# zju3dv/RelightableAvatar

Hardware: AMD Instinct MI355X
Metric: rays_per_sec (higher is better)
Workload: dtype f16

## Files before the change

### include/relightableavatar.h

```cpp
#ifndef RELIGHTABLEAVATAR_H
#define RELIGHTABLEAVATAR_H

#include <stddef.h>
#include <stdint.h>

#ifdef __cplusplus
extern "C" {
#endif

#define RA_ABI_VERSION 9
#define RA_N_LIGHTS_MAX 512

typedef struct ra_ctx ra_ctx;

const char* ra_last_error(void);
int ra_abi_version(void);

int ra_ctx_create(ra_ctx** out, int device);
int ra_ctx_destroy(ra_ctx* ctx);

typedef struct ra_config {
    int   xyz_res, sdf_res, view_res;
    int   n_bones;
    int   relight;
// ... 97 lines not shown
    int   no_visibility, local_visibility;
    int   premultiply;
    int   n_boxes;
    const float* boxes;
    const int*   box_start;
} ra_sphere_params;

int ra_render_sphere_chunk(ra_ctx* ctx, const float* ray_o, const float* ray_d, const float* near_,
                           const float* far_, int P, const float* bbox_host6,
                           const float* probe_dev, int probe_h, int probe_w,
                           const ra_sphere_params* p, const ra_render_out* out, void* stream);

int ra_gather_rays(int device, const long long* idx_dev, int n, const float* ray_o, const float* ray_d, const float* near_, const float* far_,
                   float* out_o, float* out_d, float* out_near, float* out_far, void* stream);

int ra_scatter_rows(int device, const float* src_dev, const long long* src_idx_dev, const long long* dst_idx_dev, long long n, int C,
                    float* dst_dev, void* stream);

int ra_begin_render(ra_ctx* ctx);

int ra_set_key_probes(ra_ctx* ctx, const float* probes_dev, int n, int probe_h, int probe_w, int accumulate, void* stream);

int ra_set_light_xyz(ra_ctx* ctx, const float* xyz_dev, void* stream);

int ra_light_visibility(ra_ctx* ctx, const float* surf, const float* norm, const float* acc, int n, const int* rows_dev, int n_rows,
                        const float* bbox_host6, const float* probe_dev, int probe_h, int probe_w, const ra_sphere_params* params,
                        float* lvis, float* ldot, void* stream);

int ra_render_volume_chunk(ra_ctx* ctx, const float* ray_o, const float* ray_d, const float* near_,
                           const float* far_, int P, int n_samples, float dist_th,
                           const ra_render_out* out, void* stream);

int ra_reshade(ra_ctx* ctx, const float* ray_o, const float* surf, const float* norm,
               const float* albedo, const float* roughness, const float* lvis, const float* ldot,
               int P, const float* probes_dev, int n_probes, int probe_h, int probe_w,
               float* rgb, float* shade, float* spec, void* stream);

int ra_reshade_backward(ra_ctx* ctx, const float* ray_o, const float* surf, const float* norm,
                        const float* albedo, const float* roughness, const float* lvis, const float* ldot, int P,
                        const float* probes_dev, int n_probes, int probe_h, int probe_w,
                        const float* d_rgb, float* d_albedo, float* d_roughness, float* d_probes, void* stream);

size_t ra_heads_param_count(const ra_ctx* ctx);
int ra_heads_get_params(ra_ctx* ctx, float* theta_dev, void* stream);
int ra_heads_forward(ra_ctx* ctx, const float* theta_dev, const float* feat_dev, int n, float* albedo_dev, float* rough_dev, void* stream);
int ra_heads_backward(ra_ctx* ctx, const float* theta_dev, const float* feat_dev, int n,
                      const float* d_albedo_dev, const float* d_rough_dev, float* d_theta_dev, void* stream);
int ra_bigpose_features(ra_ctx* ctx, const float* bpts_dev, int n, float* feat_dev, void* stream);

int ra_canonical_features(ra_ctx* ctx, const float* cpts_dev, int n, float* feat_dev, void* stream);
int ra_gaussian_entropy(ra_ctx* ctx, const float* x_dev, int n, const float* d_value_dev, float* value_dev, float* d_x_dev, void* stream);

int ra_reshade_ground(ra_ctx* ctx, const float* ray_d, const float* albedo_map, const float* lvis, const float* ldot, int P,
                      const float* probes_dev, int n_probes, int probe_h, int probe_w, const float* images_dev, int image_h, int image_w,
                      int attach_envmap, float* rgb, float* albedo, float* shade, float* spec, void* stream);

typedef struct ra_counters {
    uint64_t n_coarse;
    uint64_t n_fine_sdf;
    uint64_t n_fine_full;
    uint64_t n_shadow_rays;
    uint64_t n_hit_pixels;
    uint64_t n_shaded;
    uint64_t n_fine_sdf_wide;
    uint64_t n_fine_sdf_comp;
} ra_counters;
int ra_get_counters(ra_ctx* ctx, ra_counters* out, void* stream);
int ra_reset_counters(ra_ctx* ctx, void* stream);

int ra_get_mlp_time(ra_ctx* ctx, float* ms, int* n_launches, void* stream);
int ra_get_kernel_time(ra_ctx* ctx, int kind, float* ms, int* n_launches, void* stream);
int ra_enable_timing(ra_ctx* ctx, int on);
typedef struct ra_gate ra_gate;
int ra_gate_create(ra_gate** out, int device);
int ra_gate_destroy(ra_gate* gate);
int ra_set_gate(ra_ctx* ctx, ra_gate* gate);

int ra_shard_plan(const unsigned char* mask, int H, int W, int world, int ground, long long P, const long long* ground_pos,
                  const long long* edges, int n_edges, unsigned char* owner, long long* order, long long* src, long long* inds,
                  long long* counts, long long* chunk_pos, long long* n_max);

int ra_set_knn_mode(ra_ctx* ctx, int use_bvh);

typedef struct ra_ground_params {
    float normal[3];
    float origin[3];
    float albedo[3];
    int attach_envmap;
    float env_r;
    float shading_multiplier;
    ra_trace_params shadow;
    float shadow_near_offset;
    int no_visibility, local_visibility;
    int n_boxes;
    const float* boxes;
    const int* box_start;
} ra_ground_params;

typedef struct ra_ground_out {
    void* rgb;
    void* surf;
    void* albedo;
    void* shade;
    void* spec;
    void* depth;
    void* lvis;
    void* ldot;
} ra_ground_out;

int ra_render_ground_chunk(ra_ctx* ctx, const float* ray_o, const float* ray_d, const float* acc, int P, const float* bbox,
                           const float* probe, int ph, int pw, const ra_ground_params* p, const ra_ground_out* out, void* stream);

int ra_blend_ground(ra_ctx* ctx, const float* ground, const float* human, const long long* inds, const float* acc, int F, int P, int C,
                    float* dst, void* stream);

int ra_gen_rays(ra_ctx* ctx, int H, int W, const double* K, const double* R, const double* T, const float* bounds, const float* bounds_dev,
                void* ray_o, void* ray_d, void* near, void* far, void* mask_at_box, int* n_rays, int* n_rays_dev, void* stream);

typedef struct ra_pose_in {
    const float *poses, *tjoints, *big_A, *Rh, *Th;
    const int* parents;
    const int* faces;
    int n_bones, n_faces, n_verts;
    const void *tverts, *weights;
    float bounds_padding;
} ra_pose_in;
typedef struct ra_pose_out {
    void *A, *joints, *tpose, *pverts, *wverts, *pnorm, *R, *pbounds, *wbounds;
    void *poses, *Th;
} ra_pose_out;
int ra_pose_frame(ra_ctx* ctx, const ra_pose_in* in, const ra_pose_out* out, void* stream);

int ra_grow_bounds(ra_ctx* ctx, float* wbounds_dev, float margin, void* stream);

int ra_shift_envmap(ra_ctx* ctx, const float* img, int H, int W, int C, float shift, float* out, void* stream);
int ra_add_light_probe(ra_ctx* ctx, float* rgb, int H, int W, const float* probe, int ph, int pw, const float* cam_R, int uH, int uW,
                       void* stream);

enum { RA_IMG_SURFACE = 3, RA_IMG_RESIDUAL = 4, RA_IMG_DEPTH = 5, RA_IMG_ALPHA = 6, RA_IMG_NORMAL = 7, RA_IMG_SPECULAR = 8,
       RA_IMG_ALBEDO = 9, RA_IMG_ROUGHNESS = 10, RA_IMG_SHADING = 11, RA_IMG_RENDERING = 12 };
typedef struct ra_image_params {
    int type, H, W;
    float bg_brightness;
    int normalize;
    int tonemap;
    float min_clip;
    float cam_R[9];
    float tbounds[6];
} ra_image_params;
int ra_map_to_image(ra_ctx* ctx, const ra_image_params* p, const float* a_dev, const float* b_dev, const float* acc_dev,
                    const long long* pix_dev, int P, float* image_dev, float* alpha_dev, void* stream);

typedef struct ra_metrics_params {
    int H, W;
    float bg_brightness;
    float data_range;
    int mse_over_rays;
    int crop_to_mask;
} ra_metrics_params;
int ra_image_metrics(ra_ctx* ctx, const ra_metrics_params* p, const float* pred_dev, const float* gt_dev, const long long* pix_dev, int P,
                     const unsigned char* mask_dev, double* out_dev , void* stream);

typedef struct ra_lpips_weights {
    const float* conv_w[5];
    const float* conv_b[5];
    const float* lin[5];
// ... 27 lines not shown
```

### relightableavatar_amd/_lib.py

```python
import ctypes as C
import os
import subprocess

_HERE = os.path.dirname(os.path.abspath(__file__))
LIB_PATH = os.environ.get('RA_LIB_PATH') or os.path.join(_HERE, 'librelightableavatar_hip.so')
_lib = None
ABI_VERSION = 9


class RaError(RuntimeError):
    pass


class ra_config(C.Structure):
    _fields_ = [('xyz_res', C.c_int), ('sdf_res', C.c_int), ('view_res', C.c_int), ('n_bones', C.c_int), ('relight', C.c_int),
                ('resd_limit', C.c_float), ('blend_radius', C.c_float), ('albedo_slope', C.c_float), ('albedo_bias', C.c_float),
                ('roughness_slope', C.c_float), ('roughness_bias', C.c_float), ('fresnel_f0', C.c_float),
                ('shading_albedo', C.c_float), ('albedo_multiplier', C.c_float), ('lambert_only', C.c_int),
                ('glossy_only', C.c_int), ('tonemapping', C.c_int), ('bg_brightness', C.c_float), ('mlp_f16', C.c_int), ('query_skip', C.c_int),
                ('k4_batch_slots', C.c_int), ('trace_precision', C.c_int), ('clip_near', C.c_float), ('clip_far', C.c_float),
                ('only_visibility', C.c_int), ('vis_shade_map', C.c_int), ('use_geodesic_filter', C.c_int), ('key_light_share', C.c_float)]


class ra_frame(C.Structure):
# ... 35 lines not shown
class ra_ground_out(C.Structure):
    _fields_ = [(k, C.c_void_p) for k in GROUND_OUT_KEYS]


class ra_pose_in(C.Structure):
    _fields_ = [(k, C.POINTER(C.c_float)) for k in ('poses', 'tjoints', 'big_A', 'Rh', 'Th')] + \
               [('parents', C.POINTER(C.c_int)), ('faces', C.POINTER(C.c_int)), ('n_bones', C.c_int), ('n_faces', C.c_int), ('n_verts', C.c_int),
                ('tverts', C.c_void_p), ('weights', C.c_void_p), ('bounds_padding', C.c_float)]


POSE_OUT_KEYS = ('A', 'joints', 'tpose', 'pverts', 'wverts', 'pnorm', 'R', 'pbounds', 'wbounds', 'poses', 'Th')


class ra_pose_out(C.Structure):
    _fields_ = [(k, C.c_void_p) for k in POSE_OUT_KEYS]


class ra_image_params(C.Structure):
    _fields_ = [('type', C.c_int), ('H', C.c_int), ('W', C.c_int), ('bg_brightness', C.c_float), ('normalize', C.c_int), ('tonemap', C.c_int),
                ('min_clip', C.c_float), ('cam_R', C.c_float * 9), ('tbounds', C.c_float * 6)]


class ra_metrics_params(C.Structure):
    _fields_ = [('H', C.c_int), ('W', C.c_int), ('bg_brightness', C.c_float), ('data_range', C.c_float), ('mse_over_rays', C.c_int),
                ('crop_to_mask', C.c_int)]


class ra_lpips_weights(C.Structure):
    _fields_ = [('conv_w', C.c_void_p * 5), ('conv_b', C.c_void_p * 5), ('lin', C.c_void_p * 5), ('shift', C.c_float * 3), ('scale', C.c_float * 3)]


class ra_counters(C.Structure):
    _fields_ = [(k, C.c_uint64) for k in ('n_coarse', 'n_fine_sdf', 'n_fine_full', 'n_shadow_rays', 'n_hit_pixels', 'n_shaded', 'n_fine_sdf_wide', 'n_fine_sdf_comp')]


SYMBOLS = {
    'ra_last_error': (C.c_char_p, []),
    'ra_abi_version': (C.c_int, []),
    'ra_default_config': (C.c_int, [C.POINTER(ra_config)]),
    'ra_shard_plan': (C.c_int, [C.c_void_p, C.c_int, C.c_int, C.c_int, C.c_int, C.c_longlong] + [C.c_void_p] * 2 + [C.c_int] + [C.c_void_p] * 7),
    'ra_ctx_create': (C.c_int, [C.POINTER(C.c_void_p), C.c_int]),
    'ra_ctx_destroy': (C.c_int, [C.c_void_p]),
    'ra_set_config': (C.c_int, [C.c_void_p, C.POINTER(ra_config)]),
    'ra_set_weight': (C.c_int, [C.c_void_p, C.c_char_p, C.c_void_p, C.c_size_t]),
    'ra_finalize_weights': (C.c_int, [C.c_void_p, C.c_void_p]),
    'ra_set_frame': (C.c_int, [C.c_void_p, C.POINTER(ra_frame), C.c_void_p]),
    'ra_hdq_sdf': (C.c_int, [C.c_void_p, C.c_void_p, C.c_int, C.c_float, C.c_int, C.c_void_p, C.c_void_p]),
    'ra_observed_sdf': (C.c_int, [C.c_void_p, C.c_void_p, C.c_int, C.c_void_p, C.c_void_p]),
    'ra_bigpose_transform': (C.c_int, [C.c_void_p, C.c_void_p, C.c_int, C.c_void_p, C.c_void_p, C.c_int, C.c_void_p, C.c_void_p]),
    'ra_raw_channels': (C.c_int, [C.c_void_p]),
    'ra_forward': (C.c_int, [C.c_void_p, C.c_void_p, C.c_void_p, C.c_int, C.c_float, C.c_void_p, C.c_void_p]),
    'ra_sphere_trace': (C.c_int, [C.c_void_p] + [C.c_void_p] * 5 + [C.c_int, C.POINTER(ra_trace_params)] + [C.c_void_p] * 5),
    'ra_render_sphere_chunk': (C.c_int, [C.c_void_p] + [C.c_void_p] * 4 + [C.c_int, C.POINTER(C.c_float), C.c_void_p, C.c_int, C.c_int,
                                         C.POINTER(ra_sphere_params), C.POINTER(ra_render_out), C.c_void_p]),
    'ra_render_volume_chunk': (C.c_int, [C.c_void_p] + [C.c_void_p] * 4 + [C.c_int, C.c_int, C.c_float, C.POINTER(ra_render_out), C.c_void_p]),
    'ra_render_ground_chunk': (C.c_int, [C.c_void_p] + [C.c_void_p] * 3 + [C.c_int, C.POINTER(C.c_float), C.c_void_p, C.c_int, C.c_int,
                                         C.POINTER(ra_ground_params), C.POINTER(ra_ground_out), C.c_void_p]),
    'ra_blend_ground': (C.c_int, [C.c_void_p] + [C.c_void_p] * 4 + [C.c_int, C.c_int, C.c_int, C.c_void_p, C.c_void_p]),
    'ra_reshade': (C.c_int, [C.c_void_p] + [C.c_void_p] * 7 + [C.c_int, C.c_void_p, C.c_int, C.c_int, C.c_int] + [C.c_void_p] * 4),
    'ra_reshade_backward': (C.c_int, [C.c_void_p] + [C.c_void_p] * 7 + [C.c_int, C.c_void_p, C.c_int, C.c_int, C.c_int] + [C.c_void_p] * 5),
    'ra_heads_get_params': (C.c_int, [C.c_void_p, C.c_void_p, C.c_void_p]),
    'ra_heads_forward': (C.c_int, [C.c_void_p, C.c_void_p, C.c_void_p, C.c_int, C.c_void_p, C.c_void_p, C.c_void_p]),
    'ra_heads_backward': (C.c_int, [C.c_void_p, C.c_void_p, C.c_void_p, C.c_int, C.c_void_p, C.c_void_p, C.c_void_p, C.c_void_p]),
    'ra_bigpose_features': (C.c_int, [C.c_void_p, C.c_void_p, C.c_int, C.c_void_p, C.c_void_p]),
    'ra_canonical_features': (C.c_int, [C.c_void_p, C.c_void_p, C.c_int, C.c_void_p, C.c_void_p]),
    'ra_gaussian_entropy': (C.c_int, [C.c_void_p, C.c_void_p, C.c_int, C.c_void_p, C.c_void_p, C.c_void_p, C.c_void_p]),
    'ra_k3cc_enabled': (C.c_int, [C.c_void_p]),
    'ra_begin_render': (C.c_int, [C.c_void_p]),
    'ra_debug_key_lights': (C.c_int, [C.c_void_p, C.c_void_p, C.c_void_p, C.c_void_p]),
    'ra_scatter_rows': (C.c_int, [C.c_int, C.c_void_p, C.c_void_p, C.c_void_p, C.c_longlong, C.c_int, C.c_void_p, C.c_void_p]),
    'ra_gather_rays': (C.c_int, [C.c_int, C.c_void_p, C.c_int] + [C.c_void_p] * 9),
    'ra_set_key_probes': (C.c_int, [C.c_void_p, C.c_void_p, C.c_int, C.c_int, C.c_int, C.c_int, C.c_void_p]),
    'ra_set_light_xyz': (C.c_int, [C.c_void_p, C.c_void_p, C.c_void_p]),
    'ra_light_visibility': (C.c_int, [C.c_void_p, C.c_void_p, C.c_void_p, C.c_void_p, C.c_int, C.c_void_p, C.c_int, C.POINTER(C.c_float), C.c_void_p,
                                      C.c_int, C.c_int, C.POINTER(ra_sphere_params), C.c_void_p, C.c_void_p, C.c_void_p]),
    'ra_reshade_ground': (C.c_int, [C.c_void_p] + [C.c_void_p] * 4 + [C.c_int, C.c_void_p, C.c_int, C.c_int, C.c_int, C.c_void_p, C.c_int, C.c_int, C.c_int] +
                          [C.c_void_p] * 5),
    'ra_get_counters': (C.c_int, [C.c_void_p, C.POINTER(ra_counters), C.c_void_p]),
    'ra_reset_counters': (C.c_int, [C.c_void_p, C.c_void_p]),
    'ra_get_mlp_time': (C.c_int, [C.c_void_p, C.POINTER(C.c_float), C.POINTER(C.c_int), C.c_void_p]),
    'ra_get_kernel_time': (C.c_int, [C.c_void_p, C.c_int, C.POINTER(C.c_float), C.POINTER(C.c_int), C.c_void_p]),
    'ra_enable_timing': (C.c_int, [C.c_void_p, C.c_int]),
    'ra_set_knn_mode': (C.c_int, [C.c_void_p, C.c_int]),
    'ra_gate_create': (C.c_int, [C.POINTER(C.c_void_p), C.c_int]),
    'ra_gate_destroy': (C.c_int, [C.c_void_p]),
    'ra_set_gate': (C.c_int, [C.c_void_p, C.c_void_p]),
    'ra_pose_frame': (C.c_int, [C.c_void_p, C.POINTER(ra_pose_in), C.POINTER(ra_pose_out), C.c_void_p]),
    'ra_grow_bounds': (C.c_int, [C.c_void_p, C.c_void_p, C.c_float, C.c_void_p]),
    'ra_shift_envmap': (C.c_int, [C.c_void_p, C.c_void_p, C.c_int, C.c_int, C.c_int, C.c_float, C.c_void_p, C.c_void_p]),
    'ra_add_light_probe': (C.c_int, [C.c_void_p, C.c_void_p, C.c_int, C.c_int, C.c_void_p, C.c_int, C.c_int, C.POINTER(C.c_float), C.c_int, C.c_int, C.c_void_p]),
    'ra_map_to_image': (C.c_int, [C.c_void_p, C.POINTER(ra_image_params)] + [C.c_void_p] * 4 + [C.c_int, C.c_void_p, C.c_void_p, C.c_void_p]),
    'ra_image_metrics': (C.c_int, [C.c_void_p, C.POINTER(ra_metrics_params), C.c_void_p, C.c_void_p, C.c_void_p, C.c_int, C.c_void_p, C.c_void_p,
                                   C.c_void_p]),
    'ra_lpips_load': (C.c_int, [C.c_void_p, C.POINTER(ra_lpips_weights), C.c_void_p]),
    'ra_lpips_loaded': (C.c_int, [C.c_void_p]),
    'ra_lpips': (C.c_int, [C.c_void_p, C.POINTER(ra_metrics_params), C.c_void_p, C.c_void_p, C.c_void_p, C.c_int, C.c_void_p, C.c_void_p, C.c_void_p]),
    'ra_lpips_features': (C.c_int, [C.c_void_p, C.c_void_p, C.c_int, C.c_int, C.c_int, C.c_void_p, C.c_void_p]),
    'ra_lpips_tile_m': (C.c_int, []),
    'ra_gen_rays': (C.c_int, [C.c_void_p, C.c_int, C.c_int] + [C.POINTER(C.c_double)] * 3 + [C.POINTER(C.c_float), C.c_void_p] + [C.c_void_p] * 5 +
                    [C.POINTER(C.c_int), C.c_void_p, C.c_void_p]),
    'ra_debug_mlp': (C.c_int, [C.c_void_p, C.c_void_p, C.c_int, C.c_void_p, C.c_void_p, C.c_void_p, C.c_void_p]),
    'ra_debug_full': (C.c_int, [C.c_void_p, C.c_void_p, C.c_int, C.c_void_p, C.c_void_p, C.c_void_p, C.c_void_p, C.c_void_p]),
    'ra_debug_aabb': (C.c_int, [C.c_void_p, C.c_void_p, C.c_void_p, C.c_int, C.POINTER(C.c_float), C.c_void_p, C.c_void_p, C.c_void_p]),
    'ra_debug_lvis': (C.c_int, [C.c_void_p, C.c_void_p, C.c_void_p, C.c_void_p, C.c_int, C.POINTER(C.c_float), C.POINTER(ra_trace_params), C.c_float,
                                C.c_void_p, C.c_void_p, C.c_void_p]),
    'ra_debug_brdf': (C.c_int, [C.c_void_p] + [C.c_void_p] * 5 + [C.c_int, C.c_int, C.c_void_p, C.c_void_p]),
    'ra_debug_bvh_ids': (C.c_int, [C.c_void_p, C.c_void_p, C.c_int, C.POINTER(C.c_int), C.c_void_p]),
    'ra_debug_hdq': (C.c_int, [C.c_void_p, C.c_void_p, C.c_int, C.c_float] + [C.c_void_p] * 7 + [C.POINTER(C.c_int), C.c_void_p]),
}

SYMBOLS_SIZE_T = {
    'ra_heads_param_count': (C.c_size_t, [C.c_void_p]),
}


def build(verbose: bool = False) -> str:
    cmd = ['make', '-C', os.path.join(_HERE, 'csrc'), '-j8']
    r = subprocess.run(cmd, capture_output=True, text=True)
    if r.returncode != 0:
        raise RaError('building the HIP extension failed:\n' + r.stdout[-4000:] + r.stderr[-4000:])
    if verbose:
        print(r.stdout[-2000:])
    return LIB_PATH


def lib():
    global _lib
    if _lib is not None:
        return _lib
    if not os.path.exists(LIB_PATH):
        raise RaError(f'{LIB_PATH} not found: build it with `python -c "import __graft_entry__ as g; g.build()"` '
                      f'(make -C relightableavatar_amd/csrc). There is no CPU fallback for the render path.')
    import torch
    L = C.CDLL(LIB_PATH)
    for name, (res, args) in list(SYMBOLS.items()) + list(SYMBOLS_SIZE_T.items()):
        fn = getattr(L, name)
        fn.restype = res
        fn.argtypes = args
    if L.ra_abi_version() != ABI_VERSION:
        raise RaError('ABI version mismatch')
    _lib = L
    return L


def check(rc: int, what: str = ''):
    if rc != 0:
        msg = lib().ra_last_error()
        raise RaError(f'{what}: {msg.decode() if msg else "unknown error"}')
```

### relightableavatar_amd/csrc/ra_api.cpp

```cpp
#include "ra_ctx.hpp"
#include <cmath>
#include <map>
#include <mutex>
#include <vector>

#include <cstring>
#include <cstdio>
#include <cstdlib>

static thread_local std::string g_err;
void ra_set_error(const std::string& msg) { g_err = msg; }

#define RA_CHECK(cond, msg)          \
    do {                             \
        if (!(cond)) {               \
            ra_set_error(msg);       \
            return 1;                \
        }                            \
    } while (0)

int DevBuf::ensure(size_t need) {
    if (need <= bytes && p) return 0;
    if (need == 0) need = 16;
    if (p) { hipDeviceSynchronize(); hipFree(p); p = nullptr; bytes = 0; }
// ... 265 lines not shown
int* next_fine_counter(ra_ctx* c, hipStream_t s) {
    if (c->fc_next >= CNT_FC_SLOTS) {
        hipMemsetAsync(icnt(c, CNT_FC0), 0, CNT_FC_SLOTS * sizeof(int), s);
        c->fc_next = 0;
        c->fc_wrapped = true;
    }
    return icnt(c, CNT_FC0 + c->fc_next++);
}

struct HintScope {
    ra_ctx* c; hipStream_t s;
    HintScope(ra_ctx* c_, hipStream_t s_) : c(c_), s(s_) {
        const int k = c->call_no++;
        if (k >= 64) { c->cur_hint = nullptr; return; }
        if ((int)c->hints.size() <= k) c->hints.resize(k + 1);
        HintSlot& h = c->hints[k];
        if (!h.ev) {
            if (hipEventCreateWithFlags(&h.ev, hipEventDisableTiming) != hipSuccess || hipHostMalloc((void**)&h.host, CNT_FC_SLOTS * sizeof(int)) != hipSuccess) {
                h.ev = nullptr; h.host = nullptr; c->cur_hint = nullptr; (void)hipGetLastError(); return;
            }
        }
        if (h.pending && hipEventQuery(h.ev) == hipSuccess) {
            h.vals.assign(h.host, h.host + h.n_pending);
            h.n_valid = h.n_pending;
            h.pending = false;
        }
        (void)hipGetLastError();
        c->cur_hint = &h;
    }
    ~HintScope() {
        HintSlot* h = c->cur_hint;
        c->cur_hint = nullptr;
        if (!h || h->pending || c->fc_next <= 0 || c->fc_wrapped) return;
        if (hipMemcpyAsync(h->host, icnt(c, CNT_FC0), (size_t)c->fc_next * sizeof(int), hipMemcpyDeviceToHost, s) != hipSuccess) return;
        if (hipEventRecord(h->ev, s) != hipSuccess) return;
        h->n_pending = c->fc_next;
        h->pending = true;
    }
};

int fine_hint(const ra_ctx* c, int k) {
    const HintSlot* h = c->cur_hint;
    return (h && !c->fc_wrapped && k < h->n_valid) ? h->vals[k] : -1;
}
int variant_size(int n, int hint) {
    if (hint < 0) return n;
    const long long v = (long long)hint + hint / 4 + 1024;
    return v < n ? (int)v : n;
}
int grid_size(int n, int nv) { return nv > n / 8 ? nv : n / 8; }

void k3_launch(ra_ctx* c, const MlpIO& io, int n, hipStream_t s, int grid_slots = 0) {
    if (c->cfg.mlp_f16) launch_mlp_sdf_stream_f16(c->host.geo, c->sarena.p, c->sarena_pairs.p, c->barena.as<float>(), c->fr, io, n, s, grid_slots);
    else launch_mlp_sdf_stream_bf16(c->host.geo, c->sarena.p, c->sarena_pairs.p, c->barena.as<float>(), c->fr, io, n, s, grid_slots);
}

enum { Q_OTHER = 0, Q_SURFACE = 1 };
bool precise(const ra_ctx* c, int what) { return c->cfg.trace_precision >= 2 || (c->cfg.trace_precision == 1 && what == Q_SURFACE); }
constexpr int KEY_LIGHTS_MAX = 48;
bool key_tier(const ra_ctx* c) { return c->cfg.trace_precision == 1 && c->cfg.key_light_share > 0.f && c->n_lights > 0; }
int key_mask_from(ra_ctx* c, const float* probe, int ph, int pw, hipStream_t s) {
    if (c->key_external) return 0;
    c->key_valid = false;
    if (!key_tier(c) || !probe) return 0;
    if (c->key_mask.ensure((size_t)c->n_lights) || c->key_share.ensure((size_t)c->n_lights * sizeof(float))) return 1;
    launch_key_lights(probe, 1, ph, pw, c->light_dir.as<float>(), c->light_area.as<float>(), c->n_lights, c->cfg.key_light_share, KEY_LIGHTS_MAX, 0,
                      c->key_share.as<float>(), c->key_mask.as<unsigned char>(), s);
    c->key_valid = true;
    return 0;
}

void fine_level(ra_ctx* c, const MlpIO& io, int n, bool comp, hipStream_t s, int hint = -1) {
    const int nv = variant_size(n, hint);
    if (comp) {
        Timer t(c, s, 3);
        launch_mlp_sdf_comp(c->host.geo, c->sarena_c.p, c->barena.as<float>(), c->fr, io, nv, s, c->k3cc_ok, grid_size(n, nv));
    } else {
        Timer t(c, s, k3_waves(nv) == 8 ? 0 : 2);
        k3_launch(c, io, nv, s, grid_size(n, nv));
    }
}

int hdq_pass(ra_ctx* c, const RaySet& rs, int n, float th, int smooth, float* sdf, hipStream_t s, int what = Q_OTHER,
             const unsigned char* key = nullptr, int n_key = 0) {
    if (n <= 0) return 0;
    int err = 0;
    int* fine_idx = c->buf<int>("fine_idx", n, &err);
    float* bpts = c->buf<float>("fine_bpts", (size_t)n * 3, &err);
    if (err) return 1;
    HdqOut out{};
    out.sdf = sdf; out.fine_count = next_fine_counter(c, s); out.fine_idx = fine_idx; out.bpts = bpts;
    const int hint = fine_hint(c, c->fc_next - 1);
    int hint2 = -1;
    if (key && n_key > 0) {
        out.key = key;
        out.fine_idx2 = c->buf<int>("fine_idx_k", n_key, &err);
        out.bpts2 = c->buf<float>("fine_bpts_k", (size_t)n_key * 3, &err);
        if (err) return 1;
        out.fine_count2 = next_fine_counter(c, s);
        hint2 = fine_hint(c, c->fc_next - 1);
    }
    out.counters = dcnt(c);
    launch_hdq_coarse(c->fr, rs, n, th, c->cfg.blend_radius, out, s, c->cfg.use_geodesic_filter != 0);
    MlpIO io{};
    io.bpts = bpts; io.idx = fine_idx; io.count = out.fine_count; io.sdf = sdf; io.dist_th = th; io.smooth = smooth;
    io.resd_limit = c->cfg.resd_limit; io.counters = dcnt(c);
    fine_level(c, io, n, precise(c, what), s, hint);
    if (out.key) {
        io.bpts = out.bpts2; io.idx = out.fine_idx2; io.count = out.fine_count2;
        fine_level(c, io, n_key, true, s, hint2);
    }
    return 0;
}

int full_query(ra_ctx* c, FullIO io, int n, hipStream_t s) {
    const bool gated = c->gate && n > 65536;
    if (gated && c->gate->armed) RA_HIP(hipStreamWaitEvent(s, c->gate->done, 0));
    struct Release {
        ra_ctx* c; hipStream_t s; bool on;
        ~Release() { if (on) { hipEventRecord(c->gate->done, s); c->gate->armed = true; } }
    } release{c, s, gated};
    Timer t(c, s, 1);
    const int batch = c->cfg.k4_batch_slots > 0 ? c->cfg.k4_batch_slots : (1 << 20);
    const int cap = n < batch ? n : batch;
    int err = 0;
    char* tape = c->buf<char>("k4_tape", mlp_full_rev_tape_bytes(cap), &err);
    if (err) {
        ra_set_error("full query: no device memory for the activation tape (" + std::to_string(mlp_full_rev_tape_bytes(cap) >> 20) +
                     " MB): lower cfg.k4_batch_slots / cfg.volume_chunk_rays");
        return 1;
    }
    const bool f16w = c->cfg.mlp_f16 != 0;
    for (int s0 = 0; s0 < n; s0 += cap) {
        io.slot0 = s0;
        io.slot_cap = n - s0 < cap ? n - s0 : cap;
        if (f16w) {
            launch_mlp_fwd_tape_f16(c->host.geo, c->fwd_arena.p, c->barena.as<float>(), c->fr, io, tape, s);
            launch_mlp_bwd_heads_f16(c->host.mat, c->host.col, c->bwd_arena.p, c->barena.as<float>(), c->shead_row.as<float>(), c->fr, io, tape, s);
        } else {
            launch_mlp_fwd_tape_bf16(c->host.geo, c->fwd_arena.p, c->barena.as<float>(), c->fr, io, tape, s);
            launch_mlp_bwd_heads_bf16(c->host.mat, c->host.col, c->bwd_arena.p, c->barena.as<float>(), c->shead_row.as<float>(), c->fr, io, tape, s);
        }
    }
    return 0;
}

int forward_pass(ra_ctx* c, const float* x, const float* v, int n, const int* n_dev, float th, float* raw, hipStream_t s) {
    if (n <= 0) return 0;
    int err = 0;
    const int C = c->cfg.relight ? 17 : 16;
    int* fine_idx = c->buf<int>("fine_idx", n, &err);
    float* bpts = c->buf<float>("fine_bpts", (size_t)n * 3, &err);
    float* mats = c->buf<float>("fine_mats", (size_t)n * 24, &err);
    float* sdf = c->buf<float>("fwd_sdf", n, &err);
    if (err) return 1;
    RaySet rs{};
    rs.mode = 0; rs.x = x; rs.n_dev = n_dev;
    HdqOut out{};
    out.sdf = sdf; out.fine_count = next_fine_counter(c, s); out.fine_idx = fine_idx; out.bpts = bpts; out.mats = mats;
    out.raw_zero = raw; out.raw_C = C;
    out.counters = dcnt(c);
    launch_hdq_coarse(c->fr, rs, n, th, c->cfg.blend_radius, out, s, c->cfg.use_geodesic_filter != 0);
    FullIO io{};
    io.bpts = bpts; io.mats = mats; io.view = v; io.idx = fine_idx; io.count = out.fine_count; io.raw = raw; io.C = C;
    io.beta = c->host.beta; io.resd_limit = c->cfg.resd_limit;
    io.albedo_slope = c->cfg.albedo_slope; io.albedo_bias = c->cfg.albedo_bias;
    io.rough_slope = c->cfg.roughness_slope; io.rough_bias = c->cfg.roughness_bias;
    io.relight = c->cfg.relight;
    io.counters = dcnt(c);
    if (full_query(c, io, n, s)) return 1;
    return 0;
}

int check_ready(ra_ctx* c, const char* who) {
    if (!c) { ra_set_error(std::string(who) + ": null ctx"); return 1; }
    if (!c->have_weights) { ra_set_error(std::string(who) + ": weights not finalized"); return 1; }
    if (!c->have_frame) { ra_set_error(std::string(who) + ": no frame set (ra_set_frame)"); return 1; }
    if (hipSetDevice(c->device) != hipSuccess) { ra_set_error(std::string(who) + ": hipSetDevice failed"); return 1; }
    return 0;
}

TraceState alloc_trace(ra_ctx* c, const char* pfx, int n, bool soft, int* err) {
    TraceState ts{};
    std::string p(pfx);
    ts.t = c->buf<float>(p + "t", n, err);
    ts.d0 = c->buf<float>(p + "d0", n, err);
// ... 78 lines not shown
    RA_CHECK(c->cfg.relight || v || n == 0, "ra_forward: the AniSDF colour net needs view directions");
    if (forward_pass(c, x, v, n, nullptr, dist_th, raw, (hipStream_t)stream)) return 1;
    RA_HIP(hipGetLastError());
    return 0;
}

int ra_sphere_trace(ra_ctx* c, const float* ray_o, const float* ray_d, const float* near_, const float* far_, const float* tan_i,
                    int n, const ra_trace_params* p, float* surf, float* occ, float* st, float* ot, void* stream) {
    if (check_ready(c, "ra_sphere_trace")) return 1;
    RA_CHECK(p && n >= 0 && (n == 0 || (ray_o && ray_d && near_ && far_)), "ra_sphere_trace: bad arguments");
    if (n == 0) return 0;
    hipStream_t s = (hipStream_t)stream;
    int err = 0;
    TraceState ts = alloc_trace(c, "tr_", n, false, &err);
    float* sdf = c->buf<float>("tr_sdf", n, &err);
    if (err) return 1;
    ts.near_ = near_; ts.far_ = far_; ts.tan_i = tan_i; ts.light = nullptr;
    launch_trace_init(ts, n, nullptr, *p, s);
    RaySet rs{};
    rs.mode = 1; rs.o = ray_o; rs.d = ray_d; rs.t = ts.t;
    rs.nn_hint = c->buf<int>("tr_nn", (size_t)n * 3, &err);
    if (err) return 1;
    for (int it = 0; it < p->iters; ++it) {
        rs.hint_valid = it > 0;
        if (hdq_pass(c, rs, n, p->dist_th, 1, sdf, s, p->soft_shadow ? Q_OTHER : Q_SURFACE)) return 1;
        launch_trace_update(ts, sdf, n, nullptr, it, *p, s);
    }
    if (occ) RA_HIP(hipMemcpyAsync(occ, ts.occ, (size_t)n * 4, hipMemcpyDeviceToDevice, s));
    if (st) RA_HIP(hipMemcpyAsync(st, ts.st, (size_t)n * 4, hipMemcpyDeviceToDevice, s));
    if (ot) RA_HIP(hipMemcpyAsync(ot, ts.ot, (size_t)n * 4, hipMemcpyDeviceToDevice, s));
    if (surf) {
        float* depth = c->buf<float>("tr_depth", n, &err);
        float* acc = c->buf<float>("tr_acc", n, &err);
        int* hidx = c->buf<int>("tr_hidx", n, &err);
        if (err) return 1;
        launch_surface_finish(ray_o, ray_d, ts.st, ts.occ, n, surf, depth, acc, hidx, icnt(c, CNT_HIT), s);
    }
    RA_HIP(hipGetLastError());
    return 0;
}

static int light_visibility_stage(ra_ctx* c, const float* surf, const float* norm_slots, const float* acc, const int* hit_idx,
                                  const int* hit_count, int P, const float* bbox, float near_offset, const ra_trace_params& shadow,
                                  int no_visibility, int local_visibility, float** lvis_out, float** ldot_out, hipStream_t s,
                                  int n_boxes = 0, const float* boxes = nullptr, const int* box_start = nullptr, const int* pix_nn = nullptr,
                                  const int* perm = nullptr, bool split_wide_groups = false) {
    int err = 0;
    const int L = c->n_lights;
    const size_t NR = (size_t)P * L;
    float* lvis = c->buf<float>("lv_lvis", NR, &err);
    float* ldot = c->buf<float>("lv_ldot", NR, &err);
    ShadowGen g{};
    g.surf = surf; g.norm = norm_slots; g.acc = acc; g.hit_idx = hit_idx; g.hit_count = hit_count; g.ldir = c->light_dir.as<float>();
    for (int k = 0; k < 6; ++k) g.bbox[k] = bbox[k];
    g.n_boxes = n_boxes > 1 ? n_boxes : 0;
    for (int j = 0; j < g.n_boxes; ++j) {
        for (int k = 0; k < 6; ++k) g.boxes[j][k] = boxes[6 * j + k];
        g.box_start[j] = box_start[j];
    }
    if (g.n_boxes) g.box_start[g.n_boxes] = box_start[g.n_boxes];
    g.perm = g.n_boxes ? perm : nullptr;
    g.near_offset = near_offset; g.L = L; g.no_visibility = no_visibility; g.local_visibility = local_visibility;
    g.split_wide_groups = split_wide_groups ? 1 : 0;
    g.lvis = lvis; g.ldot = ldot;
    const bool traced = !(no_visibility || local_visibility);
    if (traced) {
        g.ray_pix = c->buf<int>("lv_pix", NR, &err);
        g.ray_light = c->buf<int>("lv_light", NR, &err);
        g.ray_slot = c->buf<int>("lv_slot", NR, &err);
        g.near_ = c->buf<float>("lv_near", NR, &err);
        g.far_ = c->buf<float>("lv_far", NR, &err);
    }
    g.ray_count = icnt(c, CNT_RAYS);
    TraceState sh{};
    float* ssdf = nullptr;
    if (traced) {
        sh = alloc_trace(c, "sh_", (int)NR, shadow.soft_shadow != 0, &err);
        ssdf = c->buf<float>("sh_sdf", NR, &err);
    }
    const bool keyed = traced && key_tier(c) && c->key_valid;
    const size_t NK = keyed ? (size_t)P * (size_t)(L < KEY_LIGHTS_MAX ? L : KEY_LIGHTS_MAX) : 0;
    if (err) return 1;
    if (c->gate && c->gate->armed) RA_HIP(hipStreamWaitEvent(s, c->gate->done, 0));
    launch_shadow_gen(g, P, s, c->cnt_zero);
    c->cnt_zero = false;
    if (traced) {
        sh.near_ = g.near_; sh.far_ = g.far_; sh.tan_i = c->light_sharp.as<float>(); sh.light = g.ray_light;
        launch_trace_init(sh, (int)NR, g.ray_count, shadow, s);
        RaySet r2{};
        r2.mode = 2; r2.o = surf; r2.t = sh.t; r2.pix = g.ray_pix; r2.light = g.ray_light; r2.ldir = c->light_dir.as<float>();
        r2.n_dev = g.ray_count;
        r2.skip = c->cfg.query_skip ? sh.stuck : nullptr;
        r2.nn_hint = c->buf<int>("lv_nn", NR * 3, &err);
        if (err) return 1;
        for (int it = 0; it < shadow.iters; ++it) {
            r2.hint_valid = it > 0;
            r2.hint_src = it == 0 ? pix_nn : nullptr;
            r2.hint_src_index = it == 0 ? g.ray_pix : nullptr;
            if (hdq_pass(c, r2, (int)NR, shadow.dist_th, 1, ssdf, s, Q_OTHER, keyed ? c->key_mask.as<unsigned char>() : nullptr, (int)NK)) return 1;
            launch_trace_update(sh, ssdf, (int)NR, g.ray_count, it, shadow, s);
        }
        launch_shadow_scatter(sh.occ, g.ray_slot, g.ray_count, (int)NR, lvis, s);
        launch_accumulate(g.ray_count, &dcnt(c)->n_shadow_rays, s);
    }
    if (c->gate) { RA_HIP(hipEventRecord(c->gate->done, s)); c->gate->armed = true; }
    *lvis_out = lvis;
    *ldot_out = ldot;
    return 0;
}

int ra_debug_key_lights(ra_ctx* c, unsigned char* key_dev, float* share_dev, void* stream) {
    RA_CHECK(c && key_dev && share_dev, "ra_debug_key_lights: null argument");
    RA_CHECK(c->key_valid && c->n_lights > 0, "ra_debug_key_lights: no key lights have been computed (ra_set_key_probes, or a render call with a probe)");
    RA_HIP(hipSetDevice(c->device));
    RA_HIP(hipMemcpyAsync(key_dev, c->key_mask.p, (size_t)c->n_lights, hipMemcpyDeviceToDevice, (hipStream_t)stream));
    RA_HIP(hipMemcpyAsync(share_dev, c->key_share.p, (size_t)c->n_lights * sizeof(float), hipMemcpyDeviceToDevice, (hipStream_t)stream));
    return 0;
}

int ra_begin_render(ra_ctx* c) {
    RA_CHECK(c, "ra_begin_render: null ctx");
    c->call_no = 0;
    return 0;
}

int ra_set_key_probes(ra_ctx* c, const float* probes, int n, int ph, int pw, int accumulate, void* stream) {
    RA_CHECK(c && n >= 0 && (n == 0 || (probes && ph > 0 && pw > 0)), "ra_set_key_probes: bad arguments");
    if (n == 0) { c->key_external = false; c->key_valid = false; return 0; }
    RA_CHECK(c->have_weights && c->n_lights > 0, "ra_set_key_probes: needs the relight network's light set (ra_finalize_weights)");
    RA_HIP(hipSetDevice(c->device));
    const bool acc = accumulate && c->key_external && c->key_valid;
    c->key_external = true;
    if (!key_tier(c)) { c->key_valid = false; return 0; }
    if (c->key_mask.ensure((size_t)c->n_lights) || c->key_share.ensure((size_t)c->n_lights * sizeof(float))) return 1;
    launch_key_lights(probes, n, ph, pw, c->light_dir.as<float>(), c->light_area.as<float>(), c->n_lights, c->cfg.key_light_share, KEY_LIGHTS_MAX,
                      acc ? 1 : 0, c->key_share.as<float>(), c->key_mask.as<unsigned char>(), (hipStream_t)stream);
    c->key_valid = true;
    RA_HIP(hipGetLastError());
    return 0;
}

int ra_render_sphere_chunk(ra_ctx* c, const float* ray_o, const float* ray_d, const float* near_, const float* far_, int P,
                           const float* bbox, const float* probe, int ph, int pw, const ra_sphere_params* p,
                           const ra_render_out* out, void* stream) {
    if (check_ready(c, "ra_render_sphere_chunk")) return 1;
    RA_CHECK(p && out && P >= 0, "ra_render_sphere_chunk: bad arguments");
    if (P == 0) return 0;
    RA_CHECK(ray_o && ray_d && near_ && far_, "ra_render_sphere_chunk: null ray arrays");
    const bool relit = p->relighting != 0;
    RA_CHECK(!relit || (c->cfg.relight && probe && bbox && c->n_lights > 0), "ra_render_sphere_chunk: relighting needs the relight network, a probe and a bbox");
    RA_CHECK(p->n_samples >= 1 && p->n_samples <= 16, "ra_render_sphere_chunk: n_samples out of range");
    RA_CHECK(!relit || (long long)P * c->n_lights < (1ll << 31), "ra_render_sphere_chunk: chunk too large (rays x lights must fit an int): lower cfg.render_chunk_size / cfg.sphere_chunk_rays");
    if (p->n_boxes > 1) {
        RA_CHECK(p->n_boxes <= RA_MAX_BOXES && p->boxes && p->box_start && bbox, "ra_render_sphere_chunk: at most 32 boxes per call, with their tables");
        RA_CHECK(p->box_start[0] == 0 && p->box_start[p->n_boxes] == P, "ra_render_sphere_chunk: box_start must run from 0 to P");
        for (int j = 0; j < p->n_boxes; ++j) RA_CHECK(p->box_start[j] <= p->box_start[j + 1], "ra_render_sphere_chunk: box_start must ascend");
    }
    hipStream_t s = (hipStream_t)stream;
    int err = 0;
    const int S = p->n_samples, C = c->cfg.relight ? 17 : 16, L = c->n_lights;
    zero_chunk_counters(c, s);
    HintScope hints(c, s);
    const int* perm = nullptr;
    if (bbox) {
        const size_t tb = sort_hits_temp_bytes(P);
        unsigned* k0 = c->buf<unsigned>("hs_k0", P, &err);
        unsigned* k1 = c->buf<unsigned>("hs_k1", P, &err);
        int* v0 = c->buf<int>("hs_v0", P, &err);
        int* pm_ = c->buf<int>("rs_perm", P, &err);
        char* tmp = c->buf<char>("hs_tmp", tb + 16, &err);
        float* so = c->buf<float>("rs_o", (size_t)P * 3, &err);
        float* sd = c->buf<float>("rs_d", (size_t)P * 3, &err);
        float* sn = c->buf<float>("rs_n", P, &err);
        float* sf = c->buf<float>("rs_f", P, &err);
        if (err) return 1;
        const float bmin[3] = {bbox[0], bbox[1], bbox[2]};
        if (launch_sort_rays(ray_o, ray_d, near_, far_, P, bmin, k0, k1, v0, pm_, tmp, tb, so, sd, sn, sf, s)) { ra_set_error("ra_render_sphere_chunk: radix sort failed"); return 1; }
        ray_o = so; ray_d = sd; near_ = sn; far_ = sf; perm = pm_;
    }
    TraceState ts = alloc_trace(c, "sf_", P, false, &err);
    float* sdf = c->buf<float>("sf_sdf", P, &err);
    float* surf = c->buf<float>("sf_surf", (size_t)P * 3, &err);
    float* depth = c->buf<float>("sf_depth", P, &err);
    float* acc = c->buf<float>("sf_acc", P, &err);
    int* hit_idx = c->buf<int>("sf_hit", P, &err);
    int* slot_of_ray = c->buf<int>("sf_slot", P, &err);
// ... 344 lines not shown

int ra_bigpose_features(ra_ctx* c, const float* bpts, int n, float* feat, void* stream) {
    if (check_ready(c, "ra_bigpose_features")) return 1;
    RA_CHECK(c->cfg.relight, "ra_bigpose_features: needs a relight ctx with weights");
    RA_CHECK(n >= 0, "ra_bigpose_features: bad sizes");
    if (n == 0) return 0;
    RA_CHECK(bpts && feat, "ra_bigpose_features: null input");
    return ra_debug_mlp(c, bpts, n, nullptr, nullptr, feat, stream);
}

int ra_canonical_features(ra_ctx* c, const float* cpts, int n, float* feat, void* stream) {
    if (heads_ready(c, "ra_canonical_features")) return 1;
    RA_CHECK(n >= 0, "ra_canonical_features: bad sizes");
    if (n == 0) return 0;
    RA_CHECK(cpts && feat, "ra_canonical_features: null input");
    RA_CHECK(c->host.fwd_arena.size() == (size_t)2080 * 512, "ra_canonical_features: the forward stream is not the 2080 fragments the kernel walks");
    hipStream_t s = (hipStream_t)stream;
    if (c->cfg.mlp_f16) launch_canonical_features_f16(c->host.geo, c->fwd_arena.p, c->barena.as<float>(), cpts, n, feat, s);
    else launch_canonical_features_bf16(c->host.geo, c->fwd_arena.p, c->barena.as<float>(), cpts, n, feat, s);
    RA_HIP(hipGetLastError());
    return 0;
}

int ra_gaussian_entropy(ra_ctx* c, const float* x, int n, const float* d_value, float* value, float* d_x, void* stream) {
    RA_CHECK(c, "ra_gaussian_entropy: null ctx");
    RA_CHECK(x && value, "ra_gaussian_entropy: null input");
    RA_CHECK(n >= 2, "ra_gaussian_entropy: bad sizes (the variance needs two rows)");
    RA_HIP(hipSetDevice(c->device));
    int err = 0;
    double* scratch = c->buf<double>("entropy", entropy_scratch_doubles(n), &err);
    if (err) return 1;
    launch_gaussian_entropy(x, n, d_value, value, d_x, scratch, (hipStream_t)stream);
    RA_HIP(hipGetLastError());
    return 0;
}

int ra_reshade_ground(ra_ctx* c, const float* ray_d, const float* albedo_map, const float* lvis, const float* ldot, int P,
                      const float* probes, int n_probes, int ph, int pw, const float* images, int ih, int iw, int attach_envmap,
                      float* rgb, float* albedo, float* shade, float* spec, void* stream) {
    RA_CHECK(c && c->have_weights && c->cfg.relight, "ra_reshade_ground: needs a relight ctx with weights");
    RA_CHECK(P >= 0 && n_probes >= 0, "ra_reshade_ground: bad sizes");
    if (P == 0 || n_probes == 0) return 0;
    RA_CHECK(ray_d && lvis && ldot && probes && ph > 0 && pw > 0, "ra_reshade_ground: null input");
    RA_CHECK(attach_envmap || albedo_map, "ra_reshade_ground: albedo_map is needed when the probe is not attached to the ground");
    RA_CHECK(!images || (ih > 0 && iw > 0), "ra_reshade_ground: bad image size");
    RA_HIP(hipSetDevice(c->device));
    GroundReshade in{};
    in.ray_d = ray_d; in.albedo_map = albedo_map; in.lvis = lvis; in.ldot = ldot;
    in.ldir = c->light_dir.as<float>(); in.light_area = c->light_area.as<float>(); in.L = c->n_lights;
    in.probes = probes; in.n_probes = n_probes; in.ph = ph; in.pw = pw; in.images = images; in.ih = ih; in.iw = iw;
    in.attach_envmap = attach_envmap; in.P = P;
    in.rgb = rgb; in.albedo = albedo; in.shade = shade; in.spec = spec;
    launch_ground_reshade(in, (hipStream_t)stream);
    c->n_shaded += (uint64_t)P * n_probes;
    RA_HIP(hipGetLastError());
    return 0;
}

int ra_get_counters(ra_ctx* c, ra_counters* out, void* stream) {
    RA_CHECK(c && out, "ra_get_counters: null argument");
    RA_HIP(hipSetDevice(c->device));
    RA_HIP(hipStreamSynchronize((hipStream_t)stream));
    unsigned long long h[8];
    RA_HIP(hipMemcpy(h, c->dcounters.p, sizeof(h), hipMemcpyDeviceToHost));
    out->n_coarse = h[0];
    out->n_fine_sdf = h[1];
    out->n_fine_full = h[2];
    out->n_shadow_rays = h[3];
    out->n_hit_pixels = h[4];
    out->n_shaded = c->n_shaded + h[4];
    out->n_fine_sdf_wide = h[5];
    out->n_fine_sdf_comp = h[6];
    return 0;
}

int ra_reset_counters(ra_ctx* c, void* stream) {
    RA_CHECK(c, "ra_reset_counters: null ctx");
    RA_HIP(hipSetDevice(c->device));
    RA_HIP(hipStreamSynchronize((hipStream_t)stream));
    RA_HIP(hipMemset(c->dcounters.p, 0, 64));
    c->n_coarse = 0;
    c->n_shaded = 0;
    c->ev_used = 0;
    return 0;
}

int ra_set_knn_mode(ra_ctx* c, int use_bvh) {
    RA_CHECK(c, "ra_set_knn_mode: null ctx");
    c->use_bvh = use_bvh != 0;
    c->have_frame = false;
    return 0;
}

static char* pin_acquire(ra_ctx* c, size_t bytes, int* slot) {
    PinRing& r = c->pin;
    if (bytes > r.slot_bytes) {
        if (r.base) {
            for (int k = 0; k < PinRing::n; ++k) if (r.used[k]) { hipEventSynchronize(r.ev[k]); r.used[k] = false; }
            hipHostFree(r.base);
            r.base = nullptr;
        }
        const size_t sb = (bytes + 4095) & ~(size_t)4095;
        if (hipHostMalloc((void**)&r.base, sb * PinRing::n, hipHostMallocDefault) != hipSuccess) { r.base = nullptr; r.slot_bytes = 0; return nullptr; }
        r.slot_bytes = sb;
        for (int k = 0; k < PinRing::n; ++k) if (!r.ev[k]) hipEventCreateWithFlags(&r.ev[k], hipEventDisableTiming);
    }
    const int k = r.next;
    r.next = (k + 1) % PinRing::n;
    if (r.used[k]) hipEventSynchronize(r.ev[k]);
    *slot = k;
    return r.base + (size_t)k * r.slot_bytes;
}
static void pin_release(ra_ctx* c, int slot, hipStream_t s) {
    hipEventRecord(c->pin.ev[slot], s);
    c->pin.used[slot] = true;
}

int ra_pose_frame(ra_ctx* c, const ra_pose_in* in, const ra_pose_out* out, void* stream) {
    RA_CHECK(c && in && out, "ra_pose_frame: null argument");
    const int J = in->n_bones, N = in->n_verts, F = in->n_faces;
    RA_CHECK(J > 0 && J <= 256 && N > 0 && F >= 0, "ra_pose_frame: bad sizes");
    RA_CHECK(in->poses && in->tjoints && in->parents && in->big_A && in->Rh && in->Th && in->tverts && in->weights, "ra_pose_frame: null input");
    RA_CHECK(!out->pnorm || (in->faces && F > 0), "ra_pose_frame: vertex normals need faces");
    hipStream_t s = (hipStream_t)stream;
    RA_HIP(hipSetDevice(c->device));
    for (int j = 1; j < J; ++j) RA_CHECK(in->parents[j] >= 0 && in->parents[j] < j, "ra_pose_frame: parents must be in topological order");
    const size_t n_in = (size_t)J * (3 + 3 + 16 + 1) + 6;
    int err = 0;
    float* dIn = c->buf<float>("pf_in", n_in, &err);
    float* dA = c->buf<float>("pf_A", (size_t)J * 16, &err);
    float* dJ = c->buf<float>("pf_J", (size_t)J * 3, &err);
    float* dR = c->buf<float>("pf_R", 12, &err);
    float* dP = c->buf<float>("pf_p", (size_t)N * 3, &err);
    float* dW = c->buf<float>("pf_w", (size_t)N * 3, &err);
    RA_CHECK(!err, "ra_pose_frame: out of device memory");
    {
        int slot = 0;
        float* st = reinterpret_cast<float*>(pin_acquire(c, n_in * sizeof(float), &slot));
        RA_CHECK(st, "ra_pose_frame: no pinned host memory for the staging ring");
        std::memcpy(st, in->poses, (size_t)J * 12);
        std::memcpy(st + 3 * J, in->tjoints, (size_t)J * 12);
        std::memcpy(st + 6 * J, in->big_A, (size_t)J * 64);
        std::memcpy(st + 22 * J, in->Rh, 12);
        std::memcpy(st + 22 * J + 3, in->Th, 12);
        std::memcpy(st + 22 * J + 6, in->parents, (size_t)J * 4);
        RA_HIP(hipMemcpyAsync(dIn, st, n_in * sizeof(float), hipMemcpyHostToDevice, s));
        pin_release(c, slot, s);
    }
    launch_bone_transforms(dIn, J, dA, dJ, dR, s);
    const float* dB = dIn + 6 * J;
    float* pv = out->pverts ? (float*)out->pverts : dP;
    float* wv = out->wverts ? (float*)out->wverts : dW;
    launch_lbs_verts((const float*)in->tverts, (const float*)in->weights, dA, dB, dR, dR + 9, N, J, (float*)out->tpose, pv, wv, s);
    if (out->pnorm) {
        unsigned long long fh = 1469598103934665603ull ^ (unsigned long long)F;
        {
            const size_t nw = (size_t)F * 3 / 2;
            unsigned long long lane[4] = {0x9e3779b97f4a7c15ull, 0xc2b2ae3d27d4eb4full, 0x165667b19e3779f9ull, 0x27d4eb2f165667c5ull};
            size_t k = 0;
            for (; k + 4 <= nw; k += 4)
                for (int l = 0; l < 4; ++l) {
                    unsigned long long w;
                    std::memcpy(&w, reinterpret_cast<const char*>(in->faces) + (k + l) * 8, 8);
                    lane[l] = (lane[l] ^ w) * 0x100000001b3ull;
                    lane[l] ^= lane[l] >> 29;
                }
// ... 462 lines not shown
```

### relightableavatar_amd/csrc/ra_ctx.hpp

```cpp
#pragma once
#include "ra_kernels.hpp"

struct HostNets {
    GeoNet geo{};
    MatNet mat{};
    ColNet col{};
    bool has_color = false;
    float beta = 0.1f;
    std::vector<uint16_t> sarena;
    std::vector<uint16_t> sarena_trim;
    std::vector<uint16_t> sarena_pairs;
    std::vector<uint16_t> sarena_c;
    std::vector<uint16_t> fwd_arena;
    std::vector<uint16_t> bwd_arena;
    int bwd_geo_frags = 0, bwd_frags = 0;
    std::vector<float> shead_row;
    std::vector<float> barena;
    std::vector<float> cond_r0, b_r0, cond_r4, b_r4, cond_c3, b_c3;
    std::vector<float> light_xyz, light_area, light_sharp;
};

struct DevBuf {
    void* p = nullptr;
    size_t bytes = 0;
    int ensure(size_t need);
    void release();
    template <typename T> T* as() const { return reinterpret_cast<T*>(p); }
};

struct ra_gate {
    int device = 0;
    hipEvent_t done = nullptr;
    bool armed = false;
};

struct PinRing {
    static constexpr int n = 8;
    char* base = nullptr;
    size_t slot_bytes = 0;
    int next = 0;
    hipEvent_t ev[n] = {};
    bool used[n] = {};
};

struct HintSlot {
    hipEvent_t ev = nullptr;
    int* host = nullptr;
    bool pending = false;
    int n_pending = 0;
    int n_valid = 0;
    std::vector<int> vals;
};

struct ra_ctx {
    int device = 0;
    std::vector<HintSlot> hints;
    int call_no = 0;
    HintSlot* cur_hint = nullptr;
    PinRing pin;
    ra_gate* gate = nullptr;
    ra_config cfg{};
    bool have_cfg = false, have_weights = false, have_frame = false;
    bool k3cc_ok = true;
    std::map<std::string, std::vector<float>> state_dict;
    std::vector<float> heads_theta;
    HostNets host;
    DevBuf sarena, sarena_pairs, sarena_c, fwd_arena, bwd_arena, shead_row, barena, cond_r0, cond_r4, cond_c3, b_r0, b_r4, b_c3, light_xyz, light_area, light_sharp, light_dir;
    int n_lights = 0;
    DevBuf light_xyz_loaded;
    DevBuf key_mask, key_share;
    bool key_valid = false;
    bool key_external = false;
    DevBuf lpips_arena;
    std::vector<float> lpips_host;
    bool lpips_loaded = false;
    FrameState fr{};
    DevBuf fR, fTh, fvertA, fpverts4, fpnorm, ftverts, fbias_r0, fbias_r4, fbias_c3, fcond, fbvh_pts, fbvh_pairs, fbvh_order;
    bool use_bvh = true;
    DevBuf adj_start, adj_list, adj_dfaces;
    unsigned long long adj_hash = 0;
    int adj_n_faces = 0, adj_n_verts = 0;
    std::map<std::string, DevBuf> scratch;
    DevBuf dcounters;
    int fc_next = 0;
    bool fc_wrapped = false;
    bool cnt_zero = false;
    uint64_t n_coarse = 0, n_shaded = 0;
    bool timing = false;
    std::vector<std::pair<hipEvent_t, hipEvent_t>> ev_pool;
    std::vector<int> ev_kind;
    size_t ev_used = 0;

    template <typename T> T* buf(const std::string& name, size_t count, int* err) {
        DevBuf& b = scratch[name];
        if (b.ensure(count * sizeof(T))) { *err = 1; return nullptr; }
        return b.as<T>();
    }
};

int ra_pack_weights(ra_ctx* ctx, std::string& err);
```

### relightableavatar_amd/csrc/ra_hdq.hip

```cpp
#include "ra_kernels.hpp"
#include <type_traits>
#include <cstdlib>

namespace {

constexpr int KNN_THREADS = 256;

#ifdef RA_COARSE_TS
__device__ long long ra_coarse_ts[64 * 64 * 16 * 8];
extern "C" int ra_coarse_read_timestamps(long long* out) { return (int)hipMemcpyFromSymbol(out, HIP_SYMBOL(ra_coarse_ts), sizeof(ra_coarse_ts)); }
#define RA_CSTAMP(k) do { if (tsp) { __builtin_amdgcn_sched_barrier(0); if ((threadIdx.x & 63) == 0) tsp[k] = __builtin_readcyclecounter(); __builtin_amdgcn_sched_barrier(0); } } while (0)
#else
#define RA_CSTAMP(k) do { } while (0)
#endif
constexpr int VT = 2048;

__device__ __forceinline__ void inv3d(const float R[9], float M[9]) {
    M[0] = R[4] * R[8] - R[7] * R[5];
    M[3] = -R[3] * R[8] + R[6] * R[5];
    M[6] = R[3] * R[7] - R[6] * R[4];
    M[1] = -R[1] * R[8] + R[7] * R[2];
    M[4] = R[0] * R[8] - R[6] * R[2];
    M[7] = -R[0] * R[7] + R[6] * R[1];
    M[2] = R[1] * R[5] - R[4] * R[2];
    M[5] = -R[0] * R[5] + R[3] * R[2];
    M[8] = R[0] * R[4] - R[3] * R[1];
    const float D = R[0] * M[0] + R[1] * M[3] + R[2] * M[6];
    const float inv = 1.f / (D + 1e-8f);
#pragma unroll
    for (int i = 0; i < 9; ++i) M[i] *= inv;
}

__device__ __forceinline__ float sgn(float x) { return (x > 0.f) ? 1.f : ((x < 0.f) ? -1.f : 0.f); }

__global__ void vert_blend_kernel(const float* __restrict__ weights, const float* __restrict__ A, const float* __restrict__ big_A,
                                  int n_verts, int n_bones, float* __restrict__ vertA) {
    const int v = blockIdx.x * blockDim.x + threadIdx.x;
    if (v >= n_verts) return;
    float acc[24];
#pragma unroll
    for (int e = 0; e < 24; ++e) acc[e] = 0.f;
    for (int j = 0; j < n_bones; ++j) {
        const float w = weights[(size_t)v * n_bones + j];
#pragma unroll
        for (int e = 0; e < 12; ++e) {
            acc[e] += w * A[j * 16 + e];
            acc[12 + e] += w * big_A[j * 16 + e];
        }
    }
#pragma unroll
    for (int e = 0; e < 24; ++e) vertA[(size_t)v * 24 + e] = acc[e];
}

__global__ void pack_verts_kernel(const float* __restrict__ pv, int n, float4* __restrict__ out) {
    const int v = blockIdx.x * blockDim.x + threadIdx.x;
    if (v < n) out[v] = make_float4(pv[3 * v], pv[3 * v + 1], pv[3 * v + 2], 0.f);
}

__global__ __launch_bounds__(256) void fold_bias_kernel(const float* __restrict__ W, int ld, int col0, int ncond, const float* __restrict__ cond,
                                                        const float* __restrict__ bias, float* __restrict__ out) {
    const int r = blockIdx.x * 4 + (threadIdx.x >> 6), lane = threadIdx.x & 63;
    if (r >= 256) return;
    const float* row = W + (size_t)r * ld + col0;
    float a = 0.f;
    for (int c = lane; c < ncond; c += 64) a = fmaf(row[c], cond[c], a);
#pragma unroll
    for (int o = 32; o > 0; o >>= 1) a += __shfl_xor(a, o);
    if (lane == 0) out[r] = bias[r] + a;
}

constexpr int BVH_THREADS = 1024;
constexpr int BVH_LEAF = 32;
constexpr int BVH_FAN = 8;
constexpr int BVH_MAXN = 16384;
constexpr int BVH_MAXL = BVH_MAXN / BVH_LEAF;
constexpr int BVH_MAXS = BVH_MAXL / BVH_FAN;

__device__ __forceinline__ unsigned expand10(unsigned v) {
    v = (v * 0x00010001u) & 0xFF0000FFu;
    v = (v * 0x00000101u) & 0x0F00F00Fu;
    v = (v * 0x00000011u) & 0xC30C30C3u;
    v = (v * 0x00000005u) & 0x49249249u;
    return v;
// ... 67 lines not shown
__global__ __launch_bounds__(BVH_THREADS) void bvh_boxes_kernel(const float4* __restrict__ pv, const int* __restrict__ order, int n,
                                                                float* __restrict__ leaves, float4* __restrict__ sbox, int nl, int ns) {
    __shared__ float lb[BVH_MAXL][6];
    const int tid = threadIdx.x, e = tid & 31;
    for (int l = tid >> 5; l < nl; l += BVH_THREADS / 32) {
        const int i = l * BVH_LEAF + e;
        float4 v = make_float4(__int_as_float(0x7f800000), __int_as_float(0x7f800000), __int_as_float(0x7f800000), __int_as_float(0x7fffffff));
        float lo[3] = {3e38f, 3e38f, 3e38f}, hi[3] = {-3e38f, -3e38f, -3e38f};
        if (i < n) {
            const int id = order[i];
            v = pv[id];
            v.w = __int_as_float(id);
            lo[0] = hi[0] = v.x; lo[1] = hi[1] = v.y; lo[2] = hi[2] = v.z;
        }
        float* soa = leaves + (size_t)l * (4 * BVH_LEAF) + e;
        soa[0] = v.x; soa[BVH_LEAF] = v.y; soa[2 * BVH_LEAF] = v.z; soa[3 * BVH_LEAF] = v.w;
#pragma unroll
        for (int c = 0; c < 3; ++c)
#pragma unroll
            for (int o = 16; o > 0; o >>= 1) { lo[c] = fminf(lo[c], __shfl_xor(lo[c], o)); hi[c] = fmaxf(hi[c], __shfl_xor(hi[c], o)); }
        if (e == 0) {
#pragma unroll
            for (int c = 0; c < 3; ++c) { lb[l][c] = lo[c]; lb[l][3 + c] = hi[c]; }
        }
    }
    __syncthreads();
    for (int sidx = tid; sidx < ns; sidx += BVH_THREADS) {
        float lo[3] = {3e38f, 3e38f, 3e38f}, hi[3] = {-3e38f, -3e38f, -3e38f};
        for (int k = 0; k < BVH_FAN; ++k) {
            const int l = sidx * BVH_FAN + k;
            if (l < nl)
#pragma unroll
                for (int c = 0; c < 3; ++c) { lo[c] = fminf(lo[c], lb[l][c]); hi[c] = fmaxf(hi[c], lb[l][3 + c]); }
        }
        sbox[2 * sidx] = make_float4(lo[0], lo[1], lo[2], 0.f);
        sbox[2 * sidx + 1] = make_float4(hi[0], hi[1], hi[2], 0.f);
        float* rec = reinterpret_cast<float*>(sbox + 2 * (size_t)ns) + (size_t)sidx * (6 * BVH_FAN);
        for (int k = 0; k < BVH_FAN; ++k) {
            const int l = sidx * BVH_FAN + k;
#pragma unroll
            for (int c = 0; c < 6; ++c) rec[12 * (k >> 1) + 2 * c + (k & 1)] = l < nl ? lb[l][c] : (c < 3 ? 3e38f : -3e38f);
        }
    }
}

template <int I, int N, typename F>
__device__ __forceinline__ void static_for(F&& f) {
    if constexpr (I < N) {
        f(std::integral_constant<int, I>{});
        static_for<I + 1, N>(f);
    }
}

template <int K>
__device__ __forceinline__ float row_bcast(float v) {
    return __int_as_float(__builtin_amdgcn_update_dpp(0, __float_as_int(v), 0x150 + K, 0xf, 0xf, false));
}

__device__ __forceinline__ float box_dist2(const float p[3], float lx, float ly, float lz, float hx, float hy, float hz) {
    const float dx = fmaxf(fmaxf(lx - p[0], p[0] - hx), 0.f);
    const float dy = fmaxf(fmaxf(ly - p[1], p[1] - hy), 0.f);
    const float dz = fmaxf(fmaxf(lz - p[2], p[2] - hz), 0.f);
    return dx * dx + dy * dy + dz * dz;
}

__device__ __forceinline__ float dist2(float dx, float dy, float dz) { return __fmaf_rn(dz, dz, __fmaf_rn(dx, dx, dy * dy)); }

__device__ __forceinline__ void knn_insert(float d, int id, float& d0, float& d1, float& d2, int& i0, int& i1, int& i2, bool dedup = false) {
    if (__builtin_expect(__ballot(d <= d2) == 0ull, 1)) return;
    bool fresh = true;
    if (dedup) fresh = (id != i0) & (id != i1) & (id != i2);
    const bool c2 = fresh && (d < d2 || (d == d2 && id < i2));
    const bool c1 = fresh && (d < d1 || (d == d1 && id < i1));
    const bool c0 = fresh && (d < d0 || (d == d0 && id < i0));
    const float nd2 = c1 ? d1 : (c2 ? d : d2);
    const int ni2 = c1 ? i1 : (c2 ? id : i2);
    const float nd1 = c0 ? d0 : (c1 ? d : d1);
    const int ni1 = c0 ? i0 : (c1 ? id : i1);
    d0 = c0 ? d : d0;
    i0 = c0 ? id : i0;
    d1 = nd1; i1 = ni1; d2 = nd2; i2 = ni2;
}

__device__ __forceinline__ void ray_point(const RaySet& rs, int i, float x[3]) {
    if (rs.mode == 0) {
        x[0] = rs.x[3 * i]; x[1] = rs.x[3 * i + 1]; x[2] = rs.x[3 * i + 2];
    } else if (rs.mode == 1) {
        const float t = rs.t[i];
        x[0] = rs.o[3 * i] + t * rs.d[3 * i];
        x[1] = rs.o[3 * i + 1] + t * rs.d[3 * i + 1];
        x[2] = rs.o[3 * i + 2] + t * rs.d[3 * i + 2];
    } else {
        const float t = rs.t[i];
        const int p = rs.pix[i], l = rs.light[i];
        x[0] = rs.o[3 * p] + t * rs.ldir[3 * l];
        x[1] = rs.o[3 * p + 1] + t * rs.ldir[3 * l + 1];
        x[2] = rs.o[3 * p + 2] + t * rs.ldir[3 * l + 2];
    }
}

template <bool BVH, int SPLIT, bool HINT = false>
__global__ __launch_bounds__(SPLIT == 1 ? KNN_THREADS : 64 * SPLIT) void hdq_coarse_kernel(FrameState fr, RaySet rs, int n_launch, float th, float inv2r2,
                                                                  HdqOut out, int dbg) {
    static_assert(SPLIT == 1 || (BVH && SPLIT >= 2 && SPLIT <= 16), "SPLIT > 1: the workgroup is SPLIT waves on the same 64 queries");
    constexpr int NT = SPLIT == 1 ? KNN_THREADS : 64 * SPLIT;
    __shared__ __attribute__((aligned(16))) unsigned char smem[BVH ? 16 : VT * 16];
#ifdef RA_COARSE_TS
    long long* tsp = blockIdx.x < 64 ? ra_coarse_ts + ((((dbg >> 8) & 63) * 64 + blockIdx.x) * 16 + (threadIdx.x >> 6)) * 8 : nullptr;
    dbg &= 255;
    if (tsp && (threadIdx.x & 63) == 0) { tsp[1] = tsp[2] = tsp[3] = tsp[4] = tsp[5] = tsp[6] = tsp[7] = 0; }
    RA_CSTAMP(0);
#endif
    const int n = rs.n_dev ? min(*rs.n_dev, n_launch) : n_launch;
    const int base = blockIdx.x * (SPLIT == 1 ? KNN_THREADS : 64);
    if (base >= n) return;
    if (blockIdx.x == 0 && threadIdx.x == 0 && out.counters) atomicAdd(&out.counters->n_coarse, (unsigned long long)n);
    const int i = base + (SPLIT == 1 ? threadIdx.x : (threadIdx.x & 63));
    const bool live_q = i < n && !(rs.skip && rs.skip[i < n ? i : 0]);
    bool live = live_q;
    if (__syncthreads_count(live_q) == 0) return;
    float x[3] = {0.f, 0.f, 0.f};
    if (live) ray_point(rs, i, x);
    const float xt[3] = {x[0] - fr.Th[0], x[1] - fr.Th[1], x[2] - fr.Th[2]};
    float p[3];
#pragma unroll
    for (int c = 0; c < 3; ++c) p[c] = xt[0] * fr.R[c] + xt[1] * fr.R[3 + c] + xt[2] * fr.R[6 + c];

    RA_CSTAMP(1);
    float d0 = 3.0e38f, d1 = 3.0e38f, d2 = 3.0e38f;
    int i0 = 0, i1 = 0, i2 = 0;
    if (dbg & 1) { d0 = 1e-4f; d1 = 2e-4f; d2 = 3e-4f; i0 = 0; i1 = 1; i2 = 2; }
    else if (BVH) {
        const int nl = fr.bvh_leaves, ns = fr.bvh_supers;
        if (!live) { d0 = d1 = d2 = -1.f; }
        const unsigned long long lm = __ballot(live);
        const int first = lm ? __ffsll((long long)lm) - 1 : 0;
        const int lane = threadIdx.x & 63;
        typedef float f2 __attribute__((ext_vector_type(2)));
        const f2 px2 = {p[0], p[0]}, py2 = {p[1], p[1]}, pz2 = {p[2], p[2]};
        constexpr bool hinted = HINT;
#ifdef RA_COARSE_TS
        int n_rare = 0;
#endif
        typedef float f8 __attribute__((ext_vector_type(8)));
        typedef float f4 __attribute__((ext_vector_type(4)));
        typedef int i4 __attribute__((ext_vector_type(4)));
        auto soa8 = [&](int off) __attribute__((always_inline)) { return *(const f8 __attribute__((address_space(4)))*)(fr.bvh_soa + off); };
        auto soa_id4 = [&](int off) __attribute__((always_inline)) { return *(const i4 __attribute__((address_space(4)))*)(fr.bvh_soa + off); };
        auto box4 = [&](int off) __attribute__((always_inline)) {
            return *(const f4 __attribute__((address_space(4)))*)(reinterpret_cast<const float*>(fr.bvh_sbox) + off);
        };
        auto box1 = [&](int off) __attribute__((always_inline)) { return reinterpret_cast<const float*>(fr.bvh_sbox)[off]; };
        auto scan_leaf = [&](int l) __attribute__((always_inline)) {
            const int L = l * (4 * BVH_LEAF);
            f8 cx = soa8(L), cy = soa8(L + BVH_LEAF), cz = soa8(L + 2 * BVH_LEAF), nx = cx, ny = cy, nz = cz;
            static_for<0, 4>([&](auto q_) {
                constexpr int q = decltype(q_)::value;
                static_for<0, 2>([&](auto g_) {
                    constexpr int g = decltype(g_)::value;
                    const f2 ax = {cx[4 * g], cx[4 * g + 1]}, ay = {cy[4 * g], cy[4 * g + 1]}, az = {cz[4 * g], cz[4 * g + 1]};
                    const f2 bx = {cx[4 * g + 2], cx[4 * g + 3]}, by = {cy[4 * g + 2], cy[4 * g + 3]}, bz = {cz[4 * g + 2], cz[4 * g + 3]};
                    const f2 dxa = px2 - ax, dya = py2 - ay, dza = pz2 - az, dxb = px2 - bx, dyb = py2 - by, dzb = pz2 - bz;
                    f2 da = dya * dya, db = dyb * dyb;
                    da = __builtin_elementwise_fma(dxa, dxa, da);
                    db = __builtin_elementwise_fma(dxb, dxb, db);
                    da = __builtin_elementwise_fma(dza, dza, da);
                    db = __builtin_elementwise_fma(dzb, dzb, db);
                    if (__builtin_expect(__ballot(fminf(fminf(da.x, da.y), fminf(db.x, db.y)) <= d2) != 0ull, 0)) {
#ifdef RA_COARSE_TS
                        ++n_rare;
#endif
                        const i4 id = soa_id4(L + 3 * BVH_LEAF + 8 * q + 4 * g);
                        knn_insert(da.x, id.x, d0, d1, d2, i0, i1, i2, hinted);
                        knn_insert(da.y, id.y, d0, d1, d2, i0, i1, i2, hinted);
                        knn_insert(db.x, id.z, d0, d1, d2, i0, i1, i2, hinted);
                        knn_insert(db.y, id.w, d0, d1, d2, i0, i1, i2, hinted);
                    }
                    if constexpr (g == 0 && q < 3) { nx = soa8(L + 8 * (q + 1)); ny = soa8(L + BVH_LEAF + 8 * (q + 1)); nz = soa8(L + 2 * BVH_LEAF + 8 * (q + 1)); }
                });
                cx = nx; cy = ny; cz = nz;
            });
        };
        int n_scan = 0, n_open = 0;
        if (lm != 0ull) {
            int seed = -1;
            if (hinted) {
                if (live) {
                    float e[3]; int h[3];
#pragma unroll
                    for (int k = 0; k < 3; ++k) {
                        h[k] = rs.hint_src ? rs.hint_src[3 * (size_t)rs.hint_src_index[i] + k] : rs.nn_hint[3 * (size_t)i + k];
                        const float4 v = fr.pverts4[h[k]];
                        e[k] = dist2(p[0] - v.x, p[1] - v.y, p[2] - v.z);
                    }
                    auto before = [&](int a, int b) { return e[a] < e[b] || (e[a] == e[b] && h[a] < h[b]); };
                    auto swap = [&](int a, int b) { const float te = e[a]; e[a] = e[b]; e[b] = te; const int th_ = h[a]; h[a] = h[b]; h[b] = th_; };
                    if (before(1, 0)) swap(0, 1);
                    if (before(2, 1)) swap(1, 2);
                    if (before(1, 0)) swap(0, 1);
                    d0 = e[0]; d1 = e[1]; d2 = e[2]; i0 = h[0]; i1 = h[1]; i2 = h[2];
                }
            } else {
                auto bc = [&](float v) __attribute__((always_inline)) { return __int_as_float(__builtin_amdgcn_readlane(__float_as_int(v), first)); };
                const float q[3] = {bc(p[0]), bc(p[1]), bc(p[2])};
                auto wave_argmin = [&](float d) __attribute__((always_inline)) {
// ... 141 lines not shown
#pragma unroll
        for (int w = 0; w < NT / 64; ++w) { const int cnt = wcount[w]; wcount[w] = tot; tot += cnt; const int c2 = wcount2[w]; wcount2[w] = tot2; tot2 += c2; }
        wcount[NT / 64] = (dbg & 8) ? base : (tot ? atomicAdd(out.fine_count, tot) : 0);
        wcount2[NT / 64] = tot2 ? atomicAdd(out.fine_count2, tot2) : 0;
    }
    __syncthreads();
    RA_CSTAMP(6);
    if (!fine || (dbg & 16)) return;
    const int slot = fine2 ? wcount2[NT / 64] + wcount2[wv] + __popcll(m2 & ((1ull << lane) - 1ull))
                           : wcount[NT / 64] + wcount[wv] + __popcll(m & ((1ull << lane) - 1ull));
    float w[3], ws = 0.f;
#pragma unroll
    for (int k = 0; k < 3; ++k) { w[k] = expf(-dk[k] * inv2r2); ws += w[k]; }
    ws += 1.1920928955078125e-07f;
    float M[24];
#pragma unroll
    for (int e = 0; e < 24; ++e) M[e] = 0.f;
#pragma unroll
    for (int k = 0; k < 3; ++k) {
        const float wk = w[k] / ws;
        const float4* src = reinterpret_cast<const float4*>(fr.vertA + (size_t)ik[k] * 24);
#pragma unroll
        for (int q = 0; q < 6; ++q) {
            const float4 a = src[q];
            M[4 * q] += wk * a.x; M[4 * q + 1] += wk * a.y; M[4 * q + 2] += wk * a.z; M[4 * q + 3] += wk * a.w;
        }
    }
    const float AR[9] = {M[0], M[1], M[2], M[4], M[5], M[6], M[8], M[9], M[10]};
    float Ai[9];
    inv3d(AR, Ai);
    const float q[3] = {p[0] - M[3], p[1] - M[7], p[2] - M[11]};
    float tp[3], bp[3];
#pragma unroll
    for (int r = 0; r < 3; ++r) tp[r] = Ai[3 * r] * q[0] + Ai[3 * r + 1] * q[1] + Ai[3 * r + 2] * q[2];
#pragma unroll
    for (int r = 0; r < 3; ++r) bp[r] = M[12 + 4 * r] * tp[0] + M[12 + 4 * r + 1] * tp[1] + M[12 + 4 * r + 2] * tp[2] + M[12 + 4 * r + 3];
    if (fine2) {
        out.fine_idx2[slot] = i;
        out.bpts2[3 * slot] = bp[0]; out.bpts2[3 * slot + 1] = bp[1]; out.bpts2[3 * slot + 2] = bp[2];
        return;
    }
    out.fine_idx[slot] = i;
    out.bpts[3 * slot] = bp[0]; out.bpts[3 * slot + 1] = bp[1]; out.bpts[3 * slot + 2] = bp[2];
    if (out.mats) {
        float4* dst = reinterpret_cast<float4*>(out.mats + (size_t)slot * 24);
#pragma unroll
        for (int qd = 0; qd < 6; ++qd) dst[qd] = make_float4(M[4 * qd], M[4 * qd + 1], M[4 * qd + 2], M[4 * qd + 3]);
    }
    if (out.dbg_bpts) {
#pragma unroll
        for (int c = 0; c < 3; ++c) { out.dbg_bpts[3 * i + c] = bp[c]; out.dbg_tpts[3 * i + c] = tp[c]; }
#pragma unroll
        for (int e = 0; e < 24; ++e) out.dbg_mats[(size_t)i * 24 + e] = M[e];
    }
}

}

void launch_vert_blend(const float* weights, const float* A, const float* big_A, int n_verts, int n_bones, float* vertA,
                       hipStream_t s) {
    hipLaunchKernelGGL(vert_blend_kernel, dim3((n_verts + 255) / 256), dim3(256), 0, s, weights, A, big_A, n_verts, n_bones, vertA);
}

void launch_pack_verts(const float* pverts, int n_verts, float4* out, hipStream_t s) {
    hipLaunchKernelGGL(pack_verts_kernel, dim3((n_verts + 255) / 256), dim3(256), 0, s, pverts, n_verts, out);
}

void launch_fold_bias(const float* W, int ld, int col0, int ncond, const float* cond, const float* bias, float* out,
                      hipStream_t s) {
    hipLaunchKernelGGL(fold_bias_kernel, dim3(64), dim3(256), 0, s, W, ld, col0, ncond, cond, bias, out);
}

int bvh_leaf_count(int n_verts) {
    if (n_verts > BVH_MAXN) return 0;
    return (n_verts + BVH_LEAF - 1) / BVH_LEAF;
}
int bvh_super_count(int n_leaves) { return (n_leaves + BVH_FAN - 1) / BVH_FAN; }

void launch_bvh_build(const float4* pverts4, int n_verts, int* order, float* leaves, float4* sbox, int n_leaves, int n_supers, hipStream_t s) {
    hipLaunchKernelGGL(bvh_rank_kernel, dim3((n_verts + 63) / 64), dim3(BVH_THREADS), 0, s, pverts4, n_verts, order);
    hipLaunchKernelGGL(bvh_boxes_kernel, dim3(1), dim3(BVH_THREADS), 0, s, pverts4, order, n_verts, leaves, sbox, n_leaves, n_supers);
}

void launch_hdq_coarse(const FrameState& fr, const RaySet& rs, int n, float th, float blend_radius, const HdqOut& out,
                       hipStream_t s, bool geodesic) {
    if (n <= 0) return;
    const float inv2r2 = 1.f / (2.f * blend_radius * blend_radius);
    const dim3 grid((n + KNN_THREADS - 1) / KNN_THREADS);
    int dbg = 0, probe = 0, split_max = 196608;
#ifdef RA_TESTING
    static const int e_dbg = getenv("RA_COARSE_DBG") ? atoi(getenv("RA_COARSE_DBG")) : 0;
    static const int e_probe = getenv("RA_COARSE_PROBE") ? atoi(getenv("RA_COARSE_PROBE")) : 0;
    static const int e_split = getenv("RA_COARSE_SPLIT_MAX") ? atoi(getenv("RA_COARSE_SPLIT_MAX")) : 196608;
    dbg = e_dbg; probe = e_probe; split_max = e_split;
#endif
    if (!geodesic) dbg |= 32;
#ifdef RA_COARSE_TS
    static int launch_no = 0;
    dbg |= (launch_no++ & 63) << 8;
#endif
    const bool hint = (rs.nn_hint != nullptr && rs.hint_valid != 0) || rs.hint_src != nullptr;
    for (int pass = probe ? 0 : 1; pass < 2; ++pass) {
        const int d = pass == 0 ? probe : dbg;
        if (fr.bvh_leaves > 0 && n <= split_max)
        {
            const int groups = (n + 63) / 64;
            if (hint) {
                if (n <= split_max / 8) hipLaunchKernelGGL((hdq_coarse_kernel<true, 16, true>), dim3(groups), dim3(1024), 0, s, fr, rs, n, th, inv2r2, out, d);
                else if (n <= split_max / 2) hipLaunchKernelGGL((hdq_coarse_kernel<true, 8, true>), dim3(groups), dim3(512), 0, s, fr, rs, n, th, inv2r2, out, d);
                else hipLaunchKernelGGL((hdq_coarse_kernel<true, 4, true>), dim3(groups), dim3(256), 0, s, fr, rs, n, th, inv2r2, out, d);
            } else {
                if (n <= split_max / 8) hipLaunchKernelGGL((hdq_coarse_kernel<true, 16>), dim3(groups), dim3(1024), 0, s, fr, rs, n, th, inv2r2, out, d);
                else if (n <= split_max / 2) hipLaunchKernelGGL((hdq_coarse_kernel<true, 8>), dim3(groups), dim3(512), 0, s, fr, rs, n, th, inv2r2, out, d);
                else hipLaunchKernelGGL((hdq_coarse_kernel<true, 4>), dim3(groups), dim3(256), 0, s, fr, rs, n, th, inv2r2, out, d);
            }
        }
        else if (fr.bvh_leaves > 0 && hint) hipLaunchKernelGGL((hdq_coarse_kernel<true, 1, true>), grid, dim3(KNN_THREADS), 0, s, fr, rs, n, th, inv2r2, out, d);
        else if (fr.bvh_leaves > 0) hipLaunchKernelGGL((hdq_coarse_kernel<true, 1>), grid, dim3(KNN_THREADS), 0, s, fr, rs, n, th, inv2r2, out, d);
        else hipLaunchKernelGGL((hdq_coarse_kernel<false, 1>), grid, dim3(KNN_THREADS), 0, s, fr, rs, n, th, inv2r2, out, d);
        if (pass == 0) hipMemsetAsync(out.fine_count, 0, sizeof(int), s);
    }
}
```

### relightableavatar_amd/csrc/ra_kernels.hpp

```cpp
#pragma once
#include "ra_common.hpp"
#include "ra_lpips_pack.hpp"

struct RaySet {
    int mode;
    const float* x;
    const float* o;
    const float* d;
    const float* t;
    const int* pix;
    const int* light;
    const float* ldir;
    const int* n_dev;
    const unsigned char* skip;
    int* nn_hint;
    int hint_valid;
    const int* hint_src;
    const int* hint_src_index;
};

struct HdqOut {
    float* sdf;
    int* fine_count;
    int* fine_idx;
    float* bpts;
    float* mats;
    const unsigned char* key;
    int* fine_count2;
    int* fine_idx2;
    float* bpts2;
    float* raw_zero;
    int raw_C;
    float* dbg_sdf_batch;
    int* dbg_nn_batch;
    float* dbg_d2;
    float* dbg_tpts;
    float* dbg_bpts;
    float* dbg_mats;
    DevCounters* counters;
};

void launch_vert_blend(const float* weights, const float* A, const float* big_A, int n_verts, int n_bones, float* vertA,
                       hipStream_t s);
void launch_pack_verts(const float* pverts, int n_verts, float4* out, hipStream_t s);
void launch_fold_bias(const float* W, int ld, int col0, int ncond, const float* cond, const float* bias, float* out,
                      hipStream_t s);
void launch_bvh_build(const float4* pverts4, int n_verts, int* order, float* leaves, float4* sbox, int n_leaves, int n_supers, hipStream_t s);
int bvh_leaf_count(int n_verts);
int bvh_super_count(int n_leaves);
void launch_hdq_coarse(const FrameState& fr, const RaySet& rs, int n, float th, float blend_radius, const HdqOut& out,
                       hipStream_t s, bool geodesic = true);

struct TraceState {
    float *t, *d0, *dt, *st, *ot, *cd, *occ, *off, *rlx;
    const float *near_, *far_;
    const float* tan_i;
    const int* light;
    unsigned char* stuck;
};
void launch_trace_init(const TraceState& ts, int n, const int* n_dev, const ra_trace_params& p, hipStream_t s);

void launch_trace_update(const TraceState& ts, const float* sdf, int n, const int* n_dev, int iter,
                         const ra_trace_params& p, hipStream_t s);

void launch_surface_finish(const float* ray_o, const float* ray_d, const float* st, const float* occ, int P, float* surf,
                           float* depth, float* acc, int* hit_idx, int* hit_count, hipStream_t s, int* slot_of_ray = nullptr,
                           bool counter_is_zero = false);
void launch_slot_index(const int* hit_idx, const int* hit_count, int P, int* slot_of_ray, hipStream_t s);
struct MapJob { const float* src; float* dst; int C; int premul; int src_full; };
constexpr int RA_MAX_MAP_JOBS = 16;
struct EmitMaps { MapJob job[RA_MAX_MAP_JOBS]; long long end[RA_MAX_MAP_JOBS]; int n_jobs; const int* slot_of_ray; const float* acc; const int* perm; int P; };
void launch_emit_maps(const EmitMaps& m, hipStream_t s);
void launch_surface_samples(const float* surf, const float* ray_d, const int* hit_idx, const int* hit_count, int P, int S,
                            float range, float* x, float* v, int* n_out, hipStream_t s);
struct SurfaceMaps {
    float *cpts, *bpts, *resd, *norm, *albedo, *rough, *rgb;
    float* valbedo;
};
void launch_surface_composite(const float* raw, int C, int S, const int* hit_count, int P, int relight, const ra_config& cfg,
                              const SurfaceMaps& m, hipStream_t s);

constexpr int RA_MAX_BOXES = 32;
struct ShadowGen {
    const float* surf;
    const float* norm;
    const float* acc;
    const int* hit_idx;
    const int* hit_count;
    const float* ldir;
    float bbox[6];
    int n_boxes;
    float boxes[RA_MAX_BOXES][6];
    int box_start[RA_MAX_BOXES + 1];
    const int* perm;
    float near_offset;
    int L;
    int no_visibility, local_visibility;
    int split_wide_groups;
    float* lvis;
    float* ldot;
    int* ray_pix;
    int* ray_light;
    int* ray_slot;
    float *near_, *far_;
    int* ray_count;
};
void launch_key_lights(const float* probes, int n, int ph, int pw, const float* ldir, const float* area, int L, float share, int kmax,
                       int accumulate, float* smax, unsigned char* key, hipStream_t s);
void launch_gather_shard_rays(const long long* idx, int n, const float* ro, const float* rd, const float* nr, const float* fr, float* so, float* sd,
                              float* sn, float* sf, hipStream_t s);
void launch_scatter_rows(const float* src, const long long* src_idx, const long long* dst_idx, long long n, int C, float* dst, hipStream_t s);
void launch_shadow_gen(const ShadowGen& g, int P, hipStream_t s, bool counter_is_zero = false);
void launch_debug_aabb(const float* o, const float* d, int n, const float* bbox6, float* nr, float* fr, hipStream_t s);
void launch_debug_brdf(const float* p2l, const float* p2c, const float* nrm, const float* alb, const float* rough, int L, int N, const ra_config& cfg,
                       float* out, hipStream_t s);
size_t sort_hits_temp_bytes(int P);
int launch_sort_hits(const float* surf, const float* acc, int P, const float* bbox_min, unsigned* keys_in, unsigned* keys_out,
                     int* vals_in, int* hit_idx_out, void* temp, size_t temp_bytes, hipStream_t s);
void launch_shadow_scatter(const float* occ, const int* ray_slot, const int* ray_count, int max_rays, float* lvis, hipStream_t s);

struct ShadeIn {
    const float* ray_o;
    const float* surf;
    const int* idx;
    const int* count;
    int n;
    const float *norm, *albedo, *rough;
    const float *lvis, *ldot;
    const float *light_xyz, *light_area;
    int L;
    const float* probes;
    int n_probes, ph, pw;
    int want_spec;
    float *rgb, *shade, *spec;
};
void launch_shade(const ShadeIn& in, const ra_config& cfg, hipStream_t s);

constexpr int SHADE_BWD_MAX_GRID = 768;
constexpr size_t SHADE_BWD_LDS_BYTES = 65536;
struct ShadeBwd {
    const float *ray_o, *surf, *norm, *albedo, *rough;
    const float* lvis;
    const float *light_xyz, *light_area; int L;
    const float* probes; int n_probes, ph, pw;
    const float* d_rgb;
    int P;
    float *d_albedo, *d_rough, *d_probes;
    float* slabs;
};
int shade_bwd_grid(int P);
int shade_bwd_probes_per_launch(int ph, int pw);
void launch_shade_bwd(const ShadeBwd& a, const ra_config& cfg, hipStream_t s);

constexpr int HEADS_PARAMS = 99332;
constexpr int HEADS_MAX_GRID = 128;
constexpr int HEADS_CHUNK = 32768;
constexpr size_t HEADS_TAPE_BYTES_PER_TILE = 163840;
constexpr size_t HEADS_W16_BYTES = 2 * 66048 * 2;
struct HeadsIO {
    const float *theta, *feat;
    int n;
    float *albedo, *rough;
    const float *d_albedo, *d_rough;
    float* d_theta;
    void* w16;
    unsigned* amax;
    void* tape;
    float* slabs;
};
int heads_grid(int n);
void launch_heads_forward(const HeadsIO& io, const ra_config& cfg, hipStream_t s);
void launch_heads_backward(const HeadsIO& io, const ra_config& cfg, hipStream_t s);

constexpr int ENTROPY_MAX_GRID = 256;
int entropy_grid(int n);
size_t entropy_scratch_doubles(int n);
void launch_gaussian_entropy(const float* x, int n, const float* d_value, float* value, float* d_x, double* scratch, hipStream_t s);

struct MetricsIO {
    const float *pred, *gt;
    const long long* pix;
    int P;
    const unsigned char* mask;
    int H, W;
    float bg, data_range;
    int mse_over_rays, crop_to_mask;
    double* out;
    void* scratch;
};
size_t metrics_scratch_bytes(int H, int W, bool ray_list);
void launch_image_metrics(const MetricsIO& io, hipStream_t s);

struct LpipsIO {
    const float *pred, *gt;
    const long long* pix;
    int P;
    const unsigned char* mask;
    int H, W;
    float bg;
    int crop_to_mask;
    double* out;
// ... 91 lines not shown
```

### relightableavatar_amd/csrc/ra_trace.hip

```cpp
#include "ra_kernels.hpp"
#include "ra_shade_dev.hpp"
#include <hipcub/hipcub.hpp>

namespace {

constexpr int TPB = 256;

__device__ __forceinline__ int live_count(const int* n_dev, int n) { return n_dev ? min(*n_dev, n) : n; }

__device__ __forceinline__ float linspace01(int s, int S) {
    if (S == 1) return 0.f;
    const float step = 1.f / (float)(S - 1);
    return (s < S / 2) ? (float)s * step : 1.f - (float)(S - 1 - s) * step;
}

__global__ void trace_init_kernel(TraceState ts, int n_launch, const int* n_dev, float offset, float relax) {
    const int i = blockIdx.x * TPB + threadIdx.x;
    if (i >= live_count(n_dev, n_launch)) return;
    const float nr = ts.near_[i], fr = ts.far_[i];
    ts.t[i] = nr;
    ts.d0[i] = 1e9f;
    ts.occ[i] = 1.f;
    if (ts.stuck) ts.stuck[i] = 0;
    if (ts.dt) ts.dt[i] = 1e9f;
    if (ts.st) ts.st[i] = fr;
    if (ts.ot) ts.ot[i] = fr;
    if (ts.cd) ts.cd[i] = 1e9f;
    if (ts.off) ts.off[i] = offset;
    if (ts.rlx) ts.rlx[i] = relax;
}

template <bool SOFT>
__global__ void trace_update_kernel(TraceState ts, const float* __restrict__ sdf, int n_launch, const int* n_dev, int iter,
                                    ra_trace_params p) {
    const int i = blockIdx.x * TPB + threadIdx.x;
    if (i >= live_count(n_dev, n_launch)) return;
    const float d1 = sdf[i];
    const float d0 = ts.d0[i];
    float t = ts.t[i];
    const float t_prev = t;
    float occ = ts.occ[i];
    const float nr = ts.near_[i], fr = ts.far_[i];
    float tan_i = p.tan_i;
    if (SOFT) {
        const float ti = ts.tan_i ? (ts.light ? ts.tan_i[ts.light[i]] : ts.tan_i[i]) : p.tan_i;
        tan_i = p.tan_i_multiplier * ti;
    }
    const float tan2 = (1.f / tan_i) * 2.f;
    float off = ts.off ? ts.off[i] : p.offset;
    float rlx = ts.rlx ? ts.rlx[i] : p.relax;
    float ot = ts.ot ? ts.ot[i] : 0.f;
    if (SOFT && p.clay_book && iter >= p.shadow_skip_iter) {
        const float dx0 = d0 + rlx * d0 + off;
        const float dx1 = d1 + rlx * d1 + off;
        const float dy = (dx1 * dx1) / (2.f * dx0);
        const float dx = (sqrtf(dx1 * dx1 - dy * dy) - off) / (1.f + rlx);
        const float den = fmaxf(fmaxf(t - dy, nr), p.eps);
        const float cls = fmaxf(dx, 0.f) / den / tan2;
        const bool msk = (cls < occ) && (dy < t) && (dx1 > 0.f) && (dx0 > 0.f) && (dx > 0.f) && (dy > 0.f) && (dy < dx0);
        if (msk) { ot = t - dy; occ = cls; }
    }
    if (iter >= p.shadow_skip_iter) {
        const float cls = fmaxf(d1, 0.f) / fmaxf(fmaxf(t, nr), p.eps) / tan2;
        if (cls < occ) { ot = t; occ = cls; }
    }
    if (!SOFT) {
        const float d1u = fabsf(d1), d0u = fabsf(d0);
        float st = ts.st[i], cd = ts.cd[i];
        const float dt = ts.dt[i];
        const float s0 = (d0 > 0.f) ? 1.f : ((d0 < 0.f) ? -1.f : 0.f);
        const float s1 = (d1 > 0.f) ? 1.f : ((d1 < 0.f) ? -1.f : 0.f);
        if (s0 != s1) {
            st = t - dt * fminf(fmaxf(d1u / (d0u + d1u + p.eps), 0.f), 1.f);
            off = 0.f;
            rlx = 0.f;
        }
        if (d1u < cd) { cd = d1u; st = t; }
        ts.st[i] = st;
        ts.cd[i] = cd;
        ts.off[i] = off;
        ts.rlx[i] = rlx;
    }
    const float dtn = d1 + rlx * d1 + off;
    t = t + dtn;
    t = fminf(t, fr);
    t = fmaxf(t, nr);
    if (ts.dt) ts.dt[i] = dtn;
    ts.t[i] = t;
    if (ts.stuck) ts.stuck[i] = (t == t_prev || (SOFT && occ == 0.f)) ? 1 : 0;
    ts.d0[i] = d1;
    ts.occ[i] = occ;
    if (ts.ot) ts.ot[i] = ot;
}

__global__ void surface_finish_kernel(const float* __restrict__ ro, const float* __restrict__ rd, const float* __restrict__ st,
                                      const float* __restrict__ occ, int P, float* __restrict__ surf, float* __restrict__ depth,
                                      float* __restrict__ acc, int* __restrict__ hit_idx, int* __restrict__ hit_count, int* __restrict__ slot_of_ray) {
    const int i = blockIdx.x * TPB + threadIdx.x;
    bool hit = false;
    if (i < P) {
        if (slot_of_ray) slot_of_ray[i] = -1;
        const float s = st[i];
        const float sx = ro[3 * i] + s * rd[3 * i], sy = ro[3 * i + 1] + s * rd[3 * i + 1], sz = ro[3 * i + 2] + s * rd[3 * i + 2];
        surf[3 * i] = sx; surf[3 * i + 1] = sy; surf[3 * i + 2] = sz;
        depth[i] = (sx - ro[3 * i]) / rd[3 * i];
        const float a = 1.f - occ[i];
        acc[i] = a;
        hit = a > 0.f;
    }
    const unsigned long long m = __ballot(hit);
    if (m == 0ull) return;
    const int lane = threadIdx.x & 63;
    int base = 0;
    if (lane == 0) base = atomicAdd(hit_count, __popcll(m));
    base = __shfl(base, 0);
    if (hit) hit_idx[base + __popcll(m & ((1ull << lane) - 1ull))] = i;
}

__device__ __forceinline__ unsigned expand10t(unsigned v) {
    v = (v * 0x00010001u) & 0xFF0000FFu;
    v = (v * 0x00000101u) & 0x0F00F00Fu;
    v = (v * 0x00000011u) & 0xC30C30C3u;
    v = (v * 0x00000005u) & 0x49249249u;
    return v;
}

__global__ void hit_keys_kernel(const float* __restrict__ surf, const float* __restrict__ acc, int P, float bx, float by, float bz,
                                unsigned* __restrict__ keys, int* __restrict__ vals) {
    const int i = blockIdx.x * TPB + threadIdx.x;
    if (i >= P) return;
    unsigned k = 0xffffffffu;
    if (acc[i] > 0.f) {
        const unsigned qx = (unsigned)fminf(fmaxf((surf[3 * i] - bx) * 256.f, 0.f), 1023.f);
        const unsigned qy = (unsigned)fminf(fmaxf((surf[3 * i + 1] - by) * 256.f, 0.f), 1023.f);
        const unsigned qz = (unsigned)fminf(fmaxf((surf[3 * i + 2] - bz) * 256.f, 0.f), 1023.f);
        k = (expand10t(qx) << 2) | (expand10t(qy) << 1) | expand10t(qz);
    }
    keys[i] = k;
    vals[i] = i;
}

__global__ void ray_keys_kernel(const float* __restrict__ ro, const float* __restrict__ rd, const float* __restrict__ nr, int P,
                                float bx, float by, float bz, const float* __restrict__ origin_dev, unsigned* __restrict__ keys,
                                int* __restrict__ vals) {
    const int i = blockIdx.x * TPB + threadIdx.x;
    if (i >= P) return;
    if (origin_dev) { bx = origin_dev[0]; by = origin_dev[1]; bz = origin_dev[2]; }
    const float t = nr[i];
    const unsigned qx = (unsigned)fminf(fmaxf((ro[3 * i] + t * rd[3 * i] - bx) * 256.f, 0.f), 1023.f);
    const unsigned qy = (unsigned)fminf(fmaxf((ro[3 * i + 1] + t * rd[3 * i + 1] - by) * 256.f, 0.f), 1023.f);
    const unsigned qz = (unsigned)fminf(fmaxf((ro[3 * i + 2] + t * rd[3 * i + 2] - bz) * 256.f, 0.f), 1023.f);
    keys[i] = (expand10t(qx) << 2) | (expand10t(qy) << 1) | expand10t(qz);
    vals[i] = i;
}

__global__ __launch_bounds__(1024) void entry_min_kernel(const float* __restrict__ ro, const float* __restrict__ rd, const float* __restrict__ nr,
                                                         int P, float* __restrict__ out) {
    __shared__ float sm_[16][3];
    float lo[3] = {3.4e38f, 3.4e38f, 3.4e38f};
    for (int i = threadIdx.x; i < P; i += 1024)
#pragma unroll
        for (int c = 0; c < 3; ++c) lo[c] = fminf(lo[c], ro[3 * i + c] + nr[i] * rd[3 * i + c]);
#pragma unroll
    for (int c = 0; c < 3; ++c)
#pragma unroll
        for (int o = 32; o > 0; o >>= 1) lo[c] = fminf(lo[c], __shfl_xor(lo[c], o));
    if ((threadIdx.x & 63) == 0)
#pragma unroll
        for (int c = 0; c < 3; ++c) sm_[threadIdx.x >> 6][c] = lo[c];
    __syncthreads();
    if (threadIdx.x < 3) {
        float a = sm_[0][threadIdx.x];
        for (int w = 1; w < 16; ++w) a = fminf(a, sm_[w][threadIdx.x]);
        out[threadIdx.x] = a;
    }
// ... 151 lines not shown
        o[0] = g.surf[3 * r]; o[1] = g.surf[3 * r + 1]; o[2] = g.surf[3 * r + 2];
        acc = g.acc[r];
    }
    constexpr int ROUNDS = SG_LIGHTS / (TPB / 64);
    constexpr int NL = ROUNDS * (TPB / 64);
    __shared__ int cnt[2][NL + 1];
    float nrv[ROUNDS], frv[ROUNDS];
    unsigned tmask = 0;
    float ext = 0.f;
    {
        float lo3[3], hi3[3];
#pragma unroll
        for (int k = 0; k < 3; ++k) { lo3[k] = hv ? o[k] : 3e38f; hi3[k] = hv ? o[k] : -3e38f; }
#pragma unroll
        for (int k = 0; k < 3; ++k)
#pragma unroll
            for (int sh = 32; sh > 0; sh >>= 1) { lo3[k] = fminf(lo3[k], __shfl_xor(lo3[k], sh)); hi3[k] = fmaxf(hi3[k], __shfl_xor(hi3[k], sh)); }
        ext = fmaxf(fmaxf(hi3[0] - lo3[0], hi3[1] - lo3[1]), hi3[2] - lo3[2]);
    }
    const bool halves = g.split_wide_groups && ext > SG_SPLIT_EXTENT;
#pragma unroll
    for (int round = 0; round < ROUNDS; ++round) {
        const int ll = round * (TPB / 64) + wv;
        const int l = lc * SG_LIGHTS + ll;
        bool trace = false;
        float nr = 0.f, fr = 0.f;
        if (hv && l < g.L) {
            const float dx = g.ldir[3 * l], dy = g.ldir[3 * l + 1], dz = g.ldir[3 * l + 2];
            const float ldot = dx * nrm[0] + dy * nrm[1] + dz * nrm[2];
            float lv;
            if (g.no_visibility) lv = 1.f;
            else if (g.local_visibility) lv = ldot > 0.f ? 1.f : 0.f;
            else {
                const bool front = (ldot > 0.f) && (acc > 0.f);
                lv = 0.f;
                if (front) {
                    const float d[3] = {dx, dy, dz};
                    aabb_near_far(box, o, d, nr, fr);
                    nr = fmaxf(nr, g.near_offset);
                    fr = fmaxf(fr, g.near_offset);
                    trace = nr < fr;
                    lv = 1.f;
                }
            }
            t_ldot[lane][ll] = ldot;
            t_lvis[lane][ll] = lv;
        }
        nrv[round] = nr; frv[round] = fr;
        if (trace) tmask |= 1u << round;
        const unsigned long long m = __ballot(trace);
        if (lane == 0) { cnt[0][ll] = __popcll(m & 0xffffffffull); cnt[1][ll] = __popcll(m >> 32); }
    }
    __syncthreads();
    if (threadIdx.x == 0) {
        int tot = 0;
        if (halves) {
            for (int hf = 0; hf < 2; ++hf)
                for (int k = 0; k < NL; ++k) { const int c = cnt[hf][k]; cnt[hf][k] = tot; tot += c; }
        } else {
            for (int k = 0; k < NL; ++k) {
                const int c0 = cnt[0][k], c1 = cnt[1][k];
                cnt[0][k] = tot; cnt[1][k] = tot + c0; tot += c0 + c1;
            }
        }
        cnt[0][NL] = tot ? atomicAdd(g.ray_count, tot) : 0;
    }
    __syncthreads();
    const int gbase = cnt[0][NL];
#pragma unroll
    for (int round = 0; round < ROUNDS; ++round) {
        const int ll = round * (TPB / 64) + wv;
        const bool trace = (tmask >> round) & 1u;
        const unsigned long long m = __ballot(trace);
        if (trace) {
            const int hf = lane >> 5;
            const unsigned mh = hf ? (unsigned)(m >> 32) : (unsigned)m;
            const int s = gbase + cnt[hf][ll] + __popc(mh & ((1u << (lane & 31)) - 1u));
            const int l = lc * SG_LIGHTS + ll;
            g.ray_pix[s] = r;
            g.ray_light[s] = l;
            g.ray_slot[s] = h * g.L + l;
            g.near_[s] = nrv[round];
            g.far_[s] = frv[round];
        }
    }
    const int col = threadIdx.x & (SG_LIGHTS - 1), l = lc * SG_LIGHTS + col;
    for (int row = threadIdx.x / SG_LIGHTS; row < 64; row += TPB / SG_LIGHTS) {
        const int hh = grp * 64 + row;
        if (hh < nh && l < g.L) {
            g.ldot[(size_t)hh * g.L + l] = t_ldot[row][col];
            g.lvis[(size_t)hh * g.L + l] = t_lvis[row][col];
        }
    }
}

__global__ void shadow_scatter_kernel(const float* __restrict__ occ, const int* __restrict__ ray_slot, const int* __restrict__ ray_count,
                                      int max_rays, float* __restrict__ lvis) {
    const int i = blockIdx.x * TPB + threadIdx.x;
    if (i >= min(*ray_count, max_rays)) return;
    lvis[ray_slot[i]] = occ[i];
}

__global__ __launch_bounds__(TPB) void key_lights_kernel(const float* __restrict__ probes, int n, int ph, int pw, const float* __restrict__ ldir,
                                                         const float* __restrict__ area, int L, float share, int kmax, int accumulate,
                                                         float* __restrict__ smax, unsigned char* __restrict__ key) {
    extern __shared__ float kl_w[];
    __shared__ float red[TPB / 64];
    for (int q = 0; q < n; ++q) {
        const float* img = probes + (size_t)q * ph * pw * 3;
        float part = 0.f;
        for (int l = threadIdx.x; l < L; l += TPB) {
            const float d[3] = {ldir[3 * l], ldir[3 * l + 1], ldir[3 * l + 2]};
            float c[3];
            sample_probe(img, ph, pw, d, c);
            float w = (c[0] + c[1] + c[2]) * (1.f / 3.f) * area[l];
            w = w > 0.f ? w : 0.f;
            kl_w[l] = w;
            part += w;
        }
#pragma unroll
        for (int sh = 32; sh > 0; sh >>= 1) part += __shfl_xor(part, sh);
        if ((threadIdx.x & 63) == 0) red[threadIdx.x >> 6] = part;
        __syncthreads();
        float total = 0.f;
#pragma unroll
        for (int k = 0; k < TPB / 64; ++k) total += red[k];
        for (int l = threadIdx.x; l < L; l += TPB) {
            const float sh_l = total > 0.f ? kl_w[l] / total : 0.f;
            smax[l] = (q == 0 && !accumulate) ? sh_l : fmaxf(smax[l], sh_l);
        }
        __syncthreads();
    }
    for (int l = threadIdx.x; l < L; l += TPB) kl_w[l] = smax[l];
    __syncthreads();
    const float thr = fmaxf(share, 4.f / (float)L);
    for (int l = threadIdx.x; l < L; l += TPB) {
        const float w = kl_w[l];
        bool cand = w >= thr;
        if (cand) {
            int rank = 0;
            for (int j = 0; j < L; ++j) rank += (kl_w[j] > w) || (kl_w[j] == w && j < l);
            cand = rank < kmax;
        }
        key[l] = (unsigned char)cand;
    }
}

__global__ void debug_brdf_kernel(const float* __restrict__ p2l, const float* __restrict__ p2c, const float* __restrict__ nrm, const float* __restrict__ alb,
                                  const float* __restrict__ rough, int L, int N, ra_config cfg, float* __restrict__ out) {
    const int i = blockIdx.x * TPB + threadIdx.x;
    if (i >= L * N) return;
    const int p = i % N;
    const float v[3] = {p2c[3 * p], p2c[3 * p + 1], p2c[3 * p + 2]}, n[3] = {nrm[3 * p], nrm[3 * p + 1], nrm[3 * p + 2]};
    const float a[3] = {alb[3 * p], alb[3 * p + 1], alb[3 * p + 2]}, l[3] = {p2l[3 * i], p2l[3 * i + 1], p2l[3 * i + 2]};
    const MfView mv = mf_view(v, n, rough[p]);
    float brdf[3], sb;
    mf_light(mv, l, a, cfg, brdf, sb);
    out[3 * i] = brdf[0]; out[3 * i + 1] = brdf[1]; out[3 * i + 2] = brdf[2];
}

constexpr int MAXP = 8;
__global__ __launch_bounds__(TPB) void shade_kernel(ShadeIn in, ra_config cfg) {
    const int n = in.count ? min(*in.count, in.n) : in.n;
    const int wave = (blockIdx.x * TPB + threadIdx.x) >> 6;
    const int lane = threadIdx.x & 63;
    if (wave >= n) return;
// ... 664 lines not shown
    hipLaunchKernelGGL(light_probe_kernel, grid_for(p.uH * p.uW), dim3(TPB), 0, s, p, probe, rgb);
}

__device__ __forceinline__ bool pixel_ray(const RayCam& c, int pix, float o[3], float d[3], float& nr, float& fr) {
    const double x = (double)(pix % c.W), y = (double)(pix / c.W);
    double pc[3], pw[3];
#pragma unroll
    for (int k = 0; k < 3; ++k) pc[k] = x * c.Kinv[3 * k] + y * c.Kinv[3 * k + 1] + c.Kinv[3 * k + 2] - c.T[k];
#pragma unroll
    for (int k = 0; k < 3; ++k) pw[k] = pc[0] * c.R[k] + pc[1] * c.R[3 + k] + pc[2] * c.R[6 + k] - c.o[k];
    const double inv = 1.0 / sqrt(pw[0] * pw[0] + pw[1] * pw[1] + pw[2] * pw[2]);
#pragma unroll
    for (int k = 0; k < 3; ++k) { d[k] = (float)(pw[k] * inv); o[k] = (float)c.o[k]; }
    const float nd = sqrtf(d[0] * d[0] + d[1] * d[1] + d[2] * d[2]);
    float t_near = -3.4e38f, t_far = 3.4e38f;
#pragma unroll
    for (int k = 0; k < 3; ++k) {
        float v = d[k] / nd;
        if (v < 1e-5f && v > -1e-10f) v = 1e-5f;
        if (v > -1e-5f && v < 1e-10f) v = -1e-5f;
        const float lo = c.bdev ? c.bdev[k] : c.bmin[k], hi = c.bdev ? c.bdev[3 + k] : c.bmax[k];
        const float t0 = (lo - o[k]) / v, t1 = (hi - o[k]) / v;
        t_near = fmaxf(t_near, fminf(t0, t1));
        t_far = fminf(t_far, fmaxf(t0, t1));
    }
    nr = t_near / nd / nd;
    fr = t_far / nd / nd;
    return t_near < t_far;
}

__global__ void ray_mask_kernel(RayCam c, unsigned char* __restrict__ mask) {
    const int i = blockIdx.x * TPB + threadIdx.x;
    if (i >= c.H * c.W) return;
    float o[3], d[3], nr, fr;
    mask[i] = pixel_ray(c, i, o, d, nr, fr) ? 1 : 0;
}

__global__ void ray_emit_kernel(RayCam c, const int* __restrict__ pix_idx, const int* __restrict__ count, float* __restrict__ ro,
                                float* __restrict__ rd, float* __restrict__ near_, float* __restrict__ far_) {
    const int i = blockIdx.x * TPB + threadIdx.x;
    if (i >= *count) return;
    float o[3], d[3], nr, fr;
    pixel_ray(c, pix_idx[i], o, d, nr, fr);
#pragma unroll
    for (int k = 0; k < 3; ++k) { ro[3 * i + k] = o[k]; rd[3 * i + k] = d[k]; }
    near_[i] = nr;
    far_[i] = fr;
}

size_t gen_rays_temp_bytes(int n) {
    size_t bytes = 0;
    hipcub::DeviceSelect::Flagged(nullptr, bytes, hipcub::CountingInputIterator<int>(0), (const unsigned char*)nullptr, (int*)nullptr, (int*)nullptr, n);
    return bytes;
}

int launch_gen_rays(const RayCam& cam, unsigned char* mask, int* pix_idx, int* count_dev, void* temp, size_t temp_bytes,
                    float* ray_o, float* ray_d, float* near, float* far, hipStream_t s) {
    const int n = cam.H * cam.W;
    if (n <= 0) { hipMemsetAsync(count_dev, 0, sizeof(int), s); return 0; }
    hipLaunchKernelGGL(ray_mask_kernel, grid_for(n), dim3(TPB), 0, s, cam, mask);
    if (hipcub::DeviceSelect::Flagged(temp, temp_bytes, hipcub::CountingInputIterator<int>(0), mask, pix_idx, count_dev, n, s) != hipSuccess) return 1;
    hipLaunchKernelGGL(ray_emit_kernel, grid_for(n), dim3(TPB), 0, s, cam, pix_idx, count_dev, ray_o, ray_d, near, far);
    return 0;
}

size_t sort_hits_temp_bytes(int P) {
    size_t bytes = 0;
    hipcub::DeviceRadixSort::SortPairs(nullptr, bytes, (const unsigned*)nullptr, (unsigned*)nullptr, (const int*)nullptr, (int*)nullptr, P);
    return bytes;
}

int launch_sort_hits(const float* surf, const float* acc, int P, const float* bbox_min, unsigned* keys_in, unsigned* keys_out,
                     int* vals_in, int* hit_idx_out, void* temp, size_t temp_bytes, hipStream_t s) {
    if (P <= 0) return 0;
    hipLaunchKernelGGL(hit_keys_kernel, grid_for(P), dim3(TPB), 0, s, surf, acc, P, bbox_min[0], bbox_min[1], bbox_min[2], keys_in, vals_in);
    return hipcub::DeviceRadixSort::SortPairs(temp, temp_bytes, keys_in, keys_out, vals_in, hit_idx_out, P, 0, 32, s) == hipSuccess ? 0 : 1;
}

void launch_shadow_scatter(const float* occ, const int* ray_slot, const int* ray_count, int max_rays, float* lvis, hipStream_t s) {
    if (max_rays <= 0) return;
    hipLaunchKernelGGL(shadow_scatter_kernel, grid_for(max_rays), dim3(TPB), 0, s, occ, ray_slot, ray_count, max_rays, lvis);
}

void launch_shade(const ShadeIn& in, const ra_config& cfg, hipStream_t s) {
    if (in.n <= 0) return;
    hipLaunchKernelGGL(shade_kernel, grid_for((long long)in.n * 64), dim3(TPB), 0, s, in, cfg);
}

void launch_scatter_maps(const int* hit_idx, const int* hit_count, int P, int premultiply, const float* acc_full, const float* src,
                         int C, float* dst, int src_full, const int* perm, hipStream_t s) {
    if (P <= 0) return;
    hipLaunchKernelGGL(scatter_maps_kernel, grid_for((long long)P * C), dim3(TPB), 0, s, hit_idx, hit_count, premultiply, acc_full, src, C, dst, src_full, perm);
}

int launch_sort_rays(const float* ro, const float* rd, const float* nr, const float* fr, int P, const float* bbox_min, unsigned* keys_in,
                     unsigned* keys_out, int* vals_in, int* perm, void* temp, size_t temp_bytes, float* so, float* sd, float* sn, float* sf,
                     hipStream_t s, float near_min, float far_max) {
    if (P <= 0) return 0;
    float* origin_dev = nullptr;
    if (!bbox_min) {
        origin_dev = reinterpret_cast<float*>(keys_out);
        hipLaunchKernelGGL(entry_min_kernel, dim3(1), dim3(1024), 0, s, ro, rd, nr, P, origin_dev);
    }
    hipLaunchKernelGGL(ray_keys_kernel, grid_for(P), dim3(TPB), 0, s, ro, rd, nr, P, bbox_min ? bbox_min[0] : 0.f, bbox_min ? bbox_min[1] : 0.f,
                       bbox_min ? bbox_min[2] : 0.f, origin_dev, keys_in, vals_in);
    if (hipcub::DeviceRadixSort::SortPairs(temp, temp_bytes, keys_in, keys_out, vals_in, perm, P, 0, 32, s) != hipSuccess) return 1;
    hipLaunchKernelGGL(gather_rays_kernel, grid_for(P), dim3(TPB), 0, s, perm, P, ro, rd, nr, fr, so, sd, sn, sf, near_min, far_max);
    return 0;
}

void launch_gather_shard_rays(const long long* idx, int n, const float* ro, const float* rd, const float* nr, const float* fr, float* so, float* sd,
                              float* sn, float* sf, hipStream_t s) {
    if (n <= 0) return;
    hipLaunchKernelGGL(gather_shard_rays_kernel, grid_for(n), dim3(TPB), 0, s, idx, n, ro, rd, nr, fr, so, sd, sn, sf);
}

void launch_scatter_rows(const float* src, const long long* src_idx, const long long* dst_idx, long long n, int C, float* dst, hipStream_t s) {
    if (n <= 0) return;
    hipLaunchKernelGGL(scatter_rows_kernel, grid_for(n * C), dim3(TPB), 0, s, src, src_idx, dst_idx, n, C, dst);
}

void launch_accumulate(const int* count, unsigned long long* dst, hipStream_t s) {
    hipLaunchKernelGGL(accumulate_kernel, dim3(1), dim3(1), 0, s, count, dst);
}

void launch_gather_rows(const int* hit_idx, const int* hit_count, int P, const float* src, int C, float* dst, hipStream_t s) {
    if (P <= 0) return;
    hipLaunchKernelGGL(gather_rows_kernel, grid_for((long long)P * C), dim3(TPB), 0, s, hit_idx, hit_count, src, C, dst);
}

__global__ void iota_kernel(int* __restrict__ idx, int n, int* __restrict__ count) {
    const int i = blockIdx.x * TPB + threadIdx.x;
    if (i == 0 && count) *count = n;
    if (i < n) idx[i] = i;
}
void launch_iota(int* idx, int n, int* count, hipStream_t s) {
    hipLaunchKernelGGL(iota_kernel, grid_for(n > 0 ? n : 1), dim3(TPB), 0, s, idx, n, count);
}

__device__ __forceinline__ void affine_inverse4(const float* A, float* o) {
#pragma unroll
    for (int r = 0; r < 3; ++r) {
#pragma unroll
        for (int c = 0; c < 3; ++c) o[4 * r + c] = A[4 * c + r];
        o[4 * r + 3] = -(A[r] * A[3] + A[4 + r] * A[7] + A[8 + r] * A[11]);
    }
#pragma unroll
    for (int c = 0; c < 4; ++c) o[12 + c] = A[12 + c];
}
__device__ __forceinline__ void matmul4(const float* A, const float* B, float* o) {
#pragma unroll
    for (int r = 0; r < 4; ++r)
#pragma unroll
        for (int c = 0; c < 4; ++c) o[4 * r + c] = A[4 * r] * B[c] + A[4 * r + 1] * B[4 + c] + A[4 * r + 2] * B[8 + c] + A[4 * r + 3] * B[12 + c];
}
__global__ void bigpose_compose_kernel(const float* __restrict__ mats, const float* __restrict__ d2, int n, float inv2r2, const float* __restrict__ R,
                                       const float* __restrict__ Th, int invert, float* __restrict__ out) {
    const int i = blockIdx.x * TPB + threadIdx.x;
    if (i >= n) return;
    float ws = 0.f;
#pragma unroll
    for (int k = 0; k < 3; ++k) ws += expf(-d2[3 * i + k] * inv2r2);
    const float sden = ws + 1.1920928955078125e-07f;
    float sb = 0.f;
#pragma unroll
    for (int k = 0; k < 3; ++k) sb += expf(-d2[3 * i + k] * inv2r2) / sden;
// ... 40 lines not shown
```

### relightableavatar_amd/engine.py

```python
import contextlib
import ctypes as C

import torch

from . import _lib
from ._lib import (check, ra_config, ra_counters, ra_frame, ra_ground_out, ra_ground_params, ra_lpips_weights, ra_metrics_params, ra_pose_in, ra_pose_out,
                   ra_render_out, ra_sphere_params, ra_trace_params)
from . import lpips_weights
from .base_utils import dotdict


def _ptr(t):
    return None if t is None else C.c_void_p(t.data_ptr())


def _f32(t: torch.Tensor, device) -> torch.Tensor:
    return t.detach().to(device=device, dtype=torch.float32).contiguous()


class RaysPending:

    def __init__(self, bufs, host, mask_host, event, H, W, keep):
        self._bufs, self._host, self._mask_host, self._event, self.H, self.W, self._keep = bufs, host, mask_host, event, H, W, keep

# ... 398 lines not shown
                raise ValueError('image_metrics: one pixel index per ray')
        if mask is not None:
            mask = mask.detach().to(device=d).reshape(-1).ne(0).to(torch.uint8).contiguous()
            if mask.numel() != H * W:
                raise ValueError('image_metrics: the mask must have H*W entries')
        if out is None:
            out = torch.empty(4, dtype=torch.float64, device=d)
        elif not (out.is_contiguous() and out.dtype == torch.float64 and out.device == d and tuple(out.shape) == (4,)):
            raise ValueError('image_metrics: out must be a contiguous float64 (4,) tensor on the engine\'s device')
        p = ra_metrics_params(H=int(H), W=int(W), bg_brightness=float(bg), data_range=float(data_range), mse_over_rays=int(bool(mse_over_rays)),
                              crop_to_mask=int(mask is not None))
        check(self.lib.ra_image_metrics(self.ctx, C.byref(p), _ptr(pred), _ptr(gt), _ptr(pix), P, _ptr(mask), _ptr(out), self.stream), 'ra_image_metrics')
        return out

    def lpips_load(self, state_dict):
        w = lpips_weights.resolve(state_dict)
        c = ra_lpips_weights()
        for k in range(lpips_weights.TAPS):
            c.conv_w[k] = w[f'conv{k}.weight'].ctypes.data
            c.conv_b[k] = w[f'conv{k}.bias'].ctypes.data
            c.lin[k] = w[f'lin{k}.weight'].ctypes.data
        for ch in range(3):
            c.shift[ch], c.scale[ch] = float(w['shift'][ch]), float(w['scale'][ch])
        check(self.lib.ra_lpips_load(self.ctx, C.byref(c), self.stream), 'ra_lpips_load')

    def lpips_loaded(self):
        return bool(self.lib.ra_lpips_loaded(self.ctx))

    def lpips(self, pred, gt, H, W, pix=None, mask=None, bg=0.0, out=None):
        d = self.device
        pred, gt = _f32(pred.reshape(-1, 3), d), _f32(gt.reshape(-1, 3), d)
        P = pred.shape[0]
        if gt.shape[0] != P:
            raise ValueError('lpips: pred and gt differ in size')
        if pix is not None:
            pix = pix.detach().to(device=d, dtype=torch.int64).reshape(-1).contiguous()
            if pix.numel() != P:
                raise ValueError('lpips: one pixel index per ray')
        if mask is not None:
            mask = mask.detach().to(device=d).reshape(-1).ne(0).to(torch.uint8).contiguous()
            if mask.numel() != H * W:
                raise ValueError('lpips: the mask must have H*W entries')
        if out is None:
            out = torch.empty(6, dtype=torch.float64, device=d)
        elif not (out.is_contiguous() and out.dtype == torch.float64 and out.device == d and tuple(out.shape) == (6,)):
            raise ValueError('lpips: out must be a contiguous float64 (6,) tensor on the engine\'s device')
        p = ra_metrics_params(H=int(H), W=int(W), bg_brightness=float(bg), data_range=1.0, mse_over_rays=0, crop_to_mask=int(mask is not None))
        check(self.lib.ra_lpips(self.ctx, C.byref(p), _ptr(pred), _ptr(gt), _ptr(pix), P, _ptr(mask), _ptr(out), self.stream), 'ra_lpips')
        return out

    def lpips_features(self, img, tap):
        d = self.device
        if img.ndim != 3 or img.shape[2] != 3:
            raise ValueError('lpips_features: img must be (H, W, 3)')
        H, W = int(img.shape[0]), int(img.shape[1])
        if min(H, W) < 31 or not 0 <= int(tap) < lpips_weights.TAPS:
            raise ValueError('lpips_features: an image below 31 x 31 has no features; tap 0..4')
        img = _f32(img, d)
        side = lambda n: (n - 7) // 4 + 1
        pool = lambda n: (n - 3) // 2 + 1
        h, w = side(H), side(W)
        for _ in range(min(int(tap), 2)):
            h, w = pool(h), pool(w)
        out = torch.empty(lpips_weights.CONV_SHAPES[int(tap)][0], h, w, device=d)
        check(self.lib.ra_lpips_features(self.ctx, _ptr(img), H, W, int(tap), _ptr(out), self.stream), 'ra_lpips_features')
        return out

    def counters(self) -> dotdict:
        c = ra_counters()
        check(self.lib.ra_get_counters(self.ctx, C.byref(c), self.stream), 'ra_get_counters')
        return dotdict({k: int(getattr(c, k)) for k, _ in ra_counters._fields_})

    def reset_counters(self):
        check(self.lib.ra_reset_counters(self.ctx, self.stream), 'ra_reset_counters')

    def set_gate(self, gate):
        check(self.lib.ra_set_gate(self.ctx, gate.handle if gate is not None else C.c_void_p()), 'ra_set_gate')
        self._gate = gate

    def set_knn_mode(self, use_bvh=True):
        check(self.lib.ra_set_knn_mode(self.ctx, int(use_bvh)), 'ra_set_knn_mode')
        self._frame_key = None

    def gen_rays(self, H, W, K, R, T, bounds, count=None):
        bufs, cnt = self._gen_rays(H, W, K, R, T, bounds, host_count=count is None)
        P = cnt if count is None else int(count)
        ro, rd, near, far, mask = bufs
        return dotdict(ray_o=ro[:P], ray_d=rd[:P], near=near[:P], far=far[:P], mask_at_box=mask.view(int(H), int(W)).bool())

    def _gen_rays(self, H, W, K, R, T, bounds, host_count, count_dev=None):
        import numpy as np
        Kd = np.ascontiguousarray(np.asarray(K, dtype=np.float64).reshape(9))
        Rd = np.ascontiguousarray(np.asarray(R, dtype=np.float64).reshape(9))
        Td = np.ascontiguousarray(np.asarray(T, dtype=np.float64).reshape(3))
        on_dev = isinstance(bounds, torch.Tensor) and bounds.is_cuda
        if on_dev:
            bdev = _f32(bounds.reshape(6), self.device)
            bd = None
        else:
            bd = np.ascontiguousarray(np.asarray(bounds.detach().cpu() if isinstance(bounds, torch.Tensor) else bounds, dtype=np.float32).reshape(6))
        n = int(H) * int(W)
        d = self.device
        ro, rd = torch.empty(n, 3, device=d), torch.empty(n, 3, device=d)
        near, far = torch.empty(n, device=d), torch.empty(n, device=d)
        mask = torch.empty(n, device=d, dtype=torch.uint8)
        cnt = C.c_int(0)
        dp = lambda a: a.ctypes.data_as(C.POINTER(C.c_double))
        check(self.lib.ra_gen_rays(self.ctx, int(H), int(W), dp(Kd), dp(Rd), dp(Td), None if bd is None else bd.ctypes.data_as(C.POINTER(C.c_float)),
                                   _ptr(bdev) if on_dev else None, _ptr(ro), _ptr(rd), _ptr(near), _ptr(far), _ptr(mask),
                                   C.byref(cnt) if host_count else None, None if count_dev is None else _ptr(count_dev), self.stream), 'ra_gen_rays')
        return (ro, rd, near, far, mask), cnt.value

    def gen_rays_async(self, H, W, K, R, T, bounds, mask_to_host=False):
        n = int(H) * int(W)
        d = self.device
        count_dev = torch.empty(1, device=d, dtype=torch.int32)
        bufs, _ = self._gen_rays(H, W, K, R, T, bounds, host_count=False, count_dev=count_dev)
        bdev = _f32(bounds.reshape(6), d) if isinstance(bounds, torch.Tensor) else torch.as_tensor(bounds, dtype=torch.float32, device=d).reshape(6)
        host = torch.empty(8, dtype=torch.float32, pin_memory=True)
        host[:1].view(torch.int32).copy_(count_dev, non_blocking=True)
        host[1:7].copy_(bdev, non_blocking=True)
        mask_host = None
        if mask_to_host:
            mask_host = torch.empty(n, dtype=torch.uint8, pin_memory=True)
            mask_host.copy_(bufs[4], non_blocking=True)
        ev = torch.cuda.Event()
        ev.record(torch.cuda.current_stream(d))
        return RaysPending(bufs, host, mask_host, ev, int(H), int(W), (count_dev, bdev))

    def pose_frame(self, poses, tjoints, parents, tverts, weights, big_A, faces, Rh, Th, padding=0.05):
        import numpy as np
        h32 = lambda a: np.ascontiguousarray(a.detach().cpu().numpy() if isinstance(a, torch.Tensor) else a, dtype=np.float32)
        hp, hj, hb, hr, ht = h32(poses).reshape(-1, 3), h32(tjoints).reshape(-1, 3), h32(big_A).reshape(-1, 16), h32(Rh).reshape(3), h32(Th).reshape(3)
        par = np.ascontiguousarray(parents.cpu().numpy() if isinstance(parents, torch.Tensor) else parents, dtype=np.int32)
        fc = np.ascontiguousarray(faces.cpu().numpy() if isinstance(faces, torch.Tensor) else faces, dtype=np.int32).reshape(-1, 3)
        d = self.device
        tv, w = _f32(tverts.reshape(-1, 3) if isinstance(tverts, torch.Tensor) else torch.as_tensor(tverts).reshape(-1, 3), d), \
            _f32(weights if isinstance(weights, torch.Tensor) else torch.as_tensor(weights), d)
        w = w.reshape(tv.shape[0], -1)
        J, N = hp.shape[0], tv.shape[0]
        o = dotdict(A=torch.empty(J, 4, 4, device=d), joints=torch.empty(J, 3, device=d), tverts=torch.empty(N, 3, device=d),
                    pverts=torch.empty(N, 3, device=d), wverts=torch.empty(N, 3, device=d), pnorm=torch.empty(N, 3, device=d),
                    R=torch.empty(3, 3, device=d), pbounds=torch.empty(2, 3, device=d), wbounds=torch.empty(2, 3, device=d),
                    poses=torch.empty(J, 3, device=d), Th=torch.empty(3, device=d))
        fp = lambda a: a.ctypes.data_as(C.POINTER(C.c_float))
        pin = ra_pose_in(poses=fp(hp), tjoints=fp(hj), big_A=fp(hb), Rh=fp(hr), Th=fp(ht), parents=par.ctypes.data_as(C.POINTER(C.c_int)),
                         faces=fc.ctypes.data_as(C.POINTER(C.c_int)), n_bones=J, n_faces=fc.shape[0], n_verts=N, tverts=_ptr(tv), weights=_ptr(w),
                         bounds_padding=float(padding))
        pout = ra_pose_out(A=_ptr(o.A), joints=_ptr(o.joints), tpose=_ptr(o.tverts), pverts=_ptr(o.pverts), wverts=_ptr(o.wverts),
                           pnorm=_ptr(o.pnorm), R=_ptr(o.R), pbounds=_ptr(o.pbounds), wbounds=_ptr(o.wbounds), poses=_ptr(o.poses), Th=_ptr(o.Th))
        check(self.lib.ra_pose_frame(self.ctx, C.byref(pin), C.byref(pout), self.stream), 'ra_pose_frame')
        return o

    def grow_bounds(self, wbounds, margin):
        assert wbounds.is_cuda and wbounds.dtype == torch.float32 and wbounds.is_contiguous() and wbounds.numel() == 6
        check(self.lib.ra_grow_bounds(self.ctx, _ptr(wbounds), float(margin), self.stream), 'ra_grow_bounds')
        torch.autograd.graph.increment_version(wbounds)
        return wbounds

    def shift_envmap(self, image, shift):
        x = _f32(image, self.device)
        lead = x.shape[:-3]
        x3 = x.reshape(x.shape[-3:])
        out = torch.empty_like(x3)
        check(self.lib.ra_shift_envmap(self.ctx, _ptr(x3), x3.shape[0], x3.shape[1], x3.shape[2], float(shift), _ptr(out), self.stream),
              'ra_shift_envmap')
# ... 94 lines not shown
```

Baseline: 9.170 million.

## Fold shadow trace init/update/scatter into neighbouring kernels

Fuses the shadow-ray trace state initialisation into the shadow generation kernel. The per-iteration sphere-trace update now runs inside the hinted BVH coarse kNN kernel, and the final update is merged with the scatter into the visibility map. The shared step logic moves to a common device header. This removes several launches and repeated global reads and writes of ray state per iteration, at the cost of more register pressure in the coarse kernel and some FMA contraction changes that can alter results slightly.

Measured after the change: 9.269 million (median of 6 runs). +1.1%, better.

```diff
diff --git a/include/relightableavatar.h b/include/relightableavatar.h
--- a/include/relightableavatar.h
+++ b/include/relightableavatar.h
@@ -203,6 +203,8 @@
 
 int ra_set_knn_mode(ra_ctx* ctx, int use_bvh);
 
+int ra_set_lvis_schedule(ra_ctx* ctx, int mode);
+
 typedef struct ra_ground_params {
     float normal[3];
     float origin[3];
diff --git a/relightableavatar_amd/_lib.py b/relightableavatar_amd/_lib.py
--- a/relightableavatar_amd/_lib.py
+++ b/relightableavatar_amd/_lib.py
@@ -141,6 +141,7 @@
     'ra_get_kernel_time': (C.c_int, [C.c_void_p, C.c_int, C.POINTER(C.c_float), C.POINTER(C.c_int), C.c_void_p]),
     'ra_enable_timing': (C.c_int, [C.c_void_p, C.c_int]),
     'ra_set_knn_mode': (C.c_int, [C.c_void_p, C.c_int]),
+    'ra_set_lvis_schedule': (C.c_int, [C.c_void_p, C.c_int]),
     'ra_gate_create': (C.c_int, [C.POINTER(C.c_void_p), C.c_int]),
     'ra_gate_destroy': (C.c_int, [C.c_void_p]),
     'ra_set_gate': (C.c_int, [C.c_void_p, C.c_void_p]),
diff --git a/relightableavatar_amd/csrc/ra_api.cpp b/relightableavatar_amd/csrc/ra_api.cpp
--- a/relightableavatar_amd/csrc/ra_api.cpp
+++ b/relightableavatar_amd/csrc/ra_api.cpp
@@ -371,7 +371,7 @@
 }
 
 int hdq_pass(ra_ctx* c, const RaySet& rs, int n, float th, int smooth, float* sdf, hipStream_t s, int what = Q_OTHER,
-             const unsigned char* key = nullptr, int n_key = 0) {
+             const unsigned char* key = nullptr, int n_key = 0, const RayUpdate* update = nullptr) {
     if (n <= 0) return 0;
     int err = 0;
     int* fine_idx = c->buf<int>("fine_idx", n, &err);
@@ -390,7 +390,11 @@
         hint2 = fine_hint(c, c->fc_next - 1);
     }
     out.counters = dcnt(c);
-    launch_hdq_coarse(c->fr, rs, n, th, c->cfg.blend_radius, out, s, c->cfg.use_geodesic_filter != 0);
+    if (update && !hdq_coarse_folds(c->fr, rs, *update)) {
+        launch_trace_update(update->ts, update->sdf, n, rs.n_dev, update->iter, update->p, s);
+        update = nullptr;
+    }
+    launch_hdq_coarse(c->fr, rs, n, th, c->cfg.blend_radius, out, s, c->cfg.use_geodesic_filter != 0, update);
     MlpIO io{};
     io.bpts = bpts; io.idx = fine_idx; io.count = out.fine_count; io.sdf = sdf; io.dist_th = th; io.smooth = smooth;
     io.resd_limit = c->cfg.resd_limit; io.counters = dcnt(c);
@@ -635,11 +639,16 @@
     const size_t NK = keyed ? (size_t)P * (size_t)(L < KEY_LIGHTS_MAX ? L : KEY_LIGHTS_MAX) : 0;
     if (err) return 1;
     if (c->gate && c->gate->armed) RA_HIP(hipStreamWaitEvent(s, c->gate->done, 0));
+    const bool folded = traced && c->lvis_schedule == 2;
+    if (folded) {
+        sh.near_ = g.near_; sh.far_ = g.far_; sh.tan_i = c->light_sharp.as<float>(); sh.ot = nullptr;
+        g.init = sh; g.init_offset = shadow.offset; g.init_relax = shadow.relax;
+    }
     launch_shadow_gen(g, P, s, c->cnt_zero);
     c->cnt_zero = false;
     if (traced) {
         sh.near_ = g.near_; sh.far_ = g.far_; sh.tan_i = c->light_sharp.as<float>(); sh.light = g.ray_light;
-        launch_trace_init(sh, (int)NR, g.ray_count, shadow, s);
+        if (!folded) launch_trace_init(sh, (int)NR, g.ray_count, shadow, s);
         RaySet r2{};
         r2.mode = 2; r2.o = surf; r2.t = sh.t; r2.pix = g.ray_pix; r2.light = g.ray_light; r2.ldir = c->light_dir.as<float>();
         r2.n_dev = g.ray_count;
@@ -650,11 +659,16 @@
             r2.hint_valid = it > 0;
             r2.hint_src = it == 0 ? pix_nn : nullptr;
             r2.hint_src_index = it == 0 ? g.ray_pix : nullptr;
-            if (hdq_pass(c, r2, (int)NR, shadow.dist_th, 1, ssdf, s, Q_OTHER, keyed ? c->key_mask.as<unsigned char>() : nullptr, (int)NK)) return 1;
-            launch_trace_update(sh, ssdf, (int)NR, g.ray_count, it, shadow, s);
+            const RayUpdate upd{sh, ssdf, it - 1, shadow};
+            if (hdq_pass(c, r2, (int)NR, shadow.dist_th, 1, ssdf, s, Q_OTHER, keyed ? c->key_mask.as<unsigned char>() : nullptr, (int)NK,
+                         folded && it > 0 ? &upd : nullptr)) return 1;
+            if (!folded) launch_trace_update(sh, ssdf, (int)NR, g.ray_count, it, shadow, s);
         }
-        launch_shadow_scatter(sh.occ, g.ray_slot, g.ray_count, (int)NR, lvis, s);
-        launch_accumulate(g.ray_count, &dcnt(c)->n_shadow_rays, s);
+        if (folded && shadow.iters > 0) launch_shadow_finish(sh, ssdf, g.ray_slot, g.ray_count, (int)NR, shadow.iters - 1, shadow, lvis, &dcnt(c)->n_shadow_rays, s);
+        else {
+            launch_shadow_scatter(sh.occ, g.ray_slot, g.ray_count, (int)NR, lvis, s);
+            launch_accumulate(g.ray_count, &dcnt(c)->n_shadow_rays, s);
+        }
     }
     if (c->gate) { RA_HIP(hipEventRecord(c->gate->done, s)); c->gate->armed = true; }
     *lvis_out = lvis;
@@ -1165,6 +1179,13 @@
     c->n_coarse = 0;
     c->n_shaded = 0;
     c->ev_used = 0;
+    return 0;
+}
+
+int ra_set_lvis_schedule(ra_ctx* c, int mode) {
+    RA_CHECK(c, "ra_set_lvis_schedule: null ctx");
+    RA_CHECK(mode == 0 || mode == 2, "ra_set_lvis_schedule: mode must be 0 (separate ray-state passes) or 2 (folded passes)");
+    c->lvis_schedule = mode;
     return 0;
 }
 
diff --git a/relightableavatar_amd/csrc/ra_ctx.hpp b/relightableavatar_amd/csrc/ra_ctx.hpp
--- a/relightableavatar_amd/csrc/ra_ctx.hpp
+++ b/relightableavatar_amd/csrc/ra_ctx.hpp
@@ -77,6 +77,7 @@
     FrameState fr{};
     DevBuf fR, fTh, fvertA, fpverts4, fpnorm, ftverts, fbias_r0, fbias_r4, fbias_c3, fcond, fbvh_pts, fbvh_pairs, fbvh_order;
     bool use_bvh = true;
+    int lvis_schedule = 2;
     DevBuf adj_start, adj_list, adj_dfaces;
     unsigned long long adj_hash = 0;
     int adj_n_faces = 0, adj_n_verts = 0;
diff --git a/relightableavatar_amd/csrc/ra_hdq.hip b/relightableavatar_amd/csrc/ra_hdq.hip
--- a/relightableavatar_amd/csrc/ra_hdq.hip
+++ b/relightableavatar_amd/csrc/ra_hdq.hip
@@ -1,4 +1,5 @@
 #include "ra_kernels.hpp"
+#include "ra_trace_step.hpp"
 #include <type_traits>
 #include <cstdlib>
 
@@ -232,16 +233,17 @@
     d1 = nd1; i1 = ni1; d2 = nd2; i2 = ni2;
 }
 
-__device__ __forceinline__ void ray_point(const RaySet& rs, int i, float x[3]) {
+template <bool HAVE_T = false>
+__device__ __forceinline__ void ray_point(const RaySet& rs, int i, float x[3], float t_new = 0.f) {
     if (rs.mode == 0) {
         x[0] = rs.x[3 * i]; x[1] = rs.x[3 * i + 1]; x[2] = rs.x[3 * i + 2];
     } else if (rs.mode == 1) {
-        const float t = rs.t[i];
+        const float t = HAVE_T ? t_new : rs.t[i];
         x[0] = rs.o[3 * i] + t * rs.d[3 * i];
         x[1] = rs.o[3 * i + 1] + t * rs.d[3 * i + 1];
         x[2] = rs.o[3 * i + 2] + t * rs.d[3 * i + 2];
     } else {
-        const float t = rs.t[i];
+        const float t = HAVE_T ? t_new : rs.t[i];
         const int p = rs.pix[i], l = rs.light[i];
         x[0] = rs.o[3 * p] + t * rs.ldir[3 * l];
         x[1] = rs.o[3 * p + 1] + t * rs.ldir[3 * l + 1];
@@ -249,10 +251,11 @@
     }
 }
 
-template <bool BVH, int SPLIT, bool HINT = false>
+template <bool BVH, int SPLIT, bool HINT = false, bool UPD = false>
 __global__ __launch_bounds__(SPLIT == 1 ? KNN_THREADS : 64 * SPLIT) void hdq_coarse_kernel(FrameState fr, RaySet rs, int n_launch, float th, float inv2r2,
-                                                                  HdqOut out, int dbg) {
+                                                                  HdqOut out, int dbg, RayUpdate upd) {
     static_assert(SPLIT == 1 || (BVH && SPLIT >= 2 && SPLIT <= 16), "SPLIT > 1: the workgroup is SPLIT waves on the same 64 queries");
+    static_assert(!UPD || (BVH && HINT), "UPD: only the hinted passes of a tracing loop");
     constexpr int NT = SPLIT == 1 ? KNN_THREADS : 64 * SPLIT;
     __shared__ __attribute__((aligned(16))) unsigned char smem[BVH ? 16 : VT * 16];
 #ifdef RA_COARSE_TS
@@ -266,11 +269,22 @@
     if (base >= n) return;
     if (blockIdx.x == 0 && threadIdx.x == 0 && out.counters) atomicAdd(&out.counters->n_coarse, (unsigned long long)n);
     const int i = base + (SPLIT == 1 ? threadIdx.x : (threadIdx.x & 63));
-    const bool live_q = i < n && !(rs.skip && rs.skip[i < n ? i : 0]);
+    bool live_q;
+    float x[3] = {0.f, 0.f, 0.f};
+    if constexpr (UPD) {
+        TraceStepOut u{};
+        if (i < n) u = trace_step<true>(upd.ts, upd.sdf, i, upd.iter, upd.p);
+        live_q = i < n && !(rs.skip && u.stuck);
+        const int n_live = __syncthreads_count(live_q);
+        if (i < n && threadIdx.x < (SPLIT == 1 ? KNN_THREADS : 64)) trace_step_store<true>(upd.ts, i, u);
+        if (n_live == 0) return;
+        if (live_q) ray_point<true>(rs, i, x, u.t);
+    } else {
+        live_q = i < n && !(rs.skip && rs.skip[i < n ? i : 0]);
+        if (__syncthreads_count(live_q) == 0) return;
+        if (live_q) ray_point(rs, i, x);
+    }
     bool live = live_q;
-    if (__syncthreads_count(live_q) == 0) return;
-    float x[3] = {0.f, 0.f, 0.f};
-    if (live) ray_point(rs, i, x);
     const float xt[3] = {x[0] - fr.Th[0], x[1] - fr.Th[1], x[2] - fr.Th[2]};
     float p[3];
 #pragma unroll
@@ -578,8 +592,25 @@
     hipLaunchKernelGGL(bvh_boxes_kernel, dim3(1), dim3(BVH_THREADS), 0, s, pverts4, order, n_verts, leaves, sbox, n_leaves, n_supers);
 }
 
+namespace {
+int coarse_probe_mode() {
+#ifdef RA_TESTING
+    static const int e_probe = getenv("RA_COARSE_PROBE") ? atoi(getenv("RA_COARSE_PROBE")) : 0;
+    return e_probe;
+#else
+    return 0;
+#endif
+}
+}
+
+bool hdq_coarse_folds(const FrameState& fr, const RaySet& rs, const RayUpdate& update) {
+    const bool hint = (rs.nn_hint != nullptr && rs.hint_valid != 0) || rs.hint_src != nullptr;
+    return update.p.soft_shadow && hint && fr.bvh_leaves > 0 && !coarse_probe_mode();
+}
+
 void launch_hdq_coarse(const FrameState& fr, const RaySet& rs, int n, float th, float blend_radius, const HdqOut& out,
-                       hipStream_t s, bool geodesic) {
+                       hipStream_t s, bool geodesic, const RayUpdate* update) {
+    const RayUpdate upd = update ? *update : RayUpdate{};
     if (n <= 0) return;
     const float inv2r2 = 1.f / (2.f * blend_radius * blend_radius);
     const dim3 grid((n + KNN_THREADS - 1) / KNN_THREADS);
@@ -596,24 +627,30 @@
     dbg |= (launch_no++ & 63) << 8;
 #endif
     const bool hint = (rs.nn_hint != nullptr && rs.hint_valid != 0) || rs.hint_src != nullptr;
+    const bool fold = update && hdq_coarse_folds(fr, rs, *update);
     for (int pass = probe ? 0 : 1; pass < 2; ++pass) {
         const int d = pass == 0 ? probe : dbg;
         if (fr.bvh_leaves > 0 && n <= split_max)
         {
             const int groups = (n + 63) / 64;
-            if (hint) {
-                if (n <= split_max / 8) hipLaunchKernelGGL((hdq_coarse_kernel<true, 16, true>), dim3(groups), dim3(1024), 0, s, fr, rs, n, th, inv2r2, out, d);
-                else if (n <= split_max / 2) hipLaunchKernelGGL((hdq_coarse_kernel<true, 8, true>), dim3(groups), dim3(512), 0, s, fr, rs, n, th, inv2r2, out, d);
-                else hipLaunchKernelGGL((hdq_coarse_kernel<true, 4, true>), dim3(groups), dim3(256), 0, s, fr, rs, n, th, inv2r2, out, d);
+            if (fold) {
+                if (n <= split_max / 8) hipLaunchKernelGGL((hdq_coarse_kernel<true, 16, true, true>), dim3(groups), dim3(1024), 0, s, fr, rs, n, th, inv2r2, out, d, upd);
+                else if (n <= split_max / 2) hipLaunchKernelGGL((hdq_coarse_kernel<true, 8, true, true>), dim3(groups), dim3(512), 0, s, fr, rs, n, th, inv2r2, out, d, upd);
+                else hipLaunchKernelGGL((hdq_coarse_kernel<true, 4, true, true>), dim3(groups), dim3(256), 0, s, fr, rs, n, th, inv2r2, out, d, upd);
+            } else if (hint) {
+                if (n <= split_max / 8) hipLaunchKernelGGL((hdq_coarse_kernel<true, 16, true>), dim3(groups), dim3(1024), 0, s, fr, rs, n, th, inv2r2, out, d, upd);
+                else if (n <= split_max / 2) hipLaunchKernelGGL((hdq_coarse_kernel<true, 8, true>), dim3(groups), dim3(512), 0, s, fr, rs, n, th, inv2r2, out, d, upd);
+                else hipLaunchKernelGGL((hdq_coarse_kernel<true, 4, true>), dim3(groups), dim3(256), 0, s, fr, rs, n, th, inv2r2, out, d, upd);
             } else {
-                if (n <= split_max / 8) hipLaunchKernelGGL((hdq_coarse_kernel<true, 16>), dim3(groups), dim3(1024), 0, s, fr, rs, n, th, inv2r2, out, d);
-                else if (n <= split_max / 2) hipLaunchKernelGGL((hdq_coarse_kernel<true, 8>), dim3(groups), dim3(512), 0, s, fr, rs, n, th, inv2r2, out, d);
-                else hipLaunchKernelGGL((hdq_coarse_kernel<true, 4>), dim3(groups), dim3(256), 0, s, fr, rs, n, th, inv2r2, out, d);
-            }
-        }
-        else if (fr.bvh_leaves > 0 && hint) hipLaunchKernelGGL((hdq_coarse_kernel<true, 1, true>), grid, dim3(KNN_THREADS), 0, s, fr, rs, n, th, inv2r2, out, d);
-        else if (fr.bvh_leaves > 0) hipLaunchKernelGGL((hdq_coarse_kernel<true, 1>), grid, dim3(KNN_THREADS), 0, s, fr, rs, n, th, inv2r2, out, d);
-        else hipLaunchKernelGGL((hdq_coarse_kernel<false, 1>), grid, dim3(KNN_THREADS), 0, s, fr, rs, n, th, inv2r2, out, d);
+                if (n <= split_max / 8) hipLaunchKernelGGL((hdq_coarse_kernel<true, 16>), dim3(groups), dim3(1024), 0, s, fr, rs, n, th, inv2r2, out, d, upd);
+                else if (n <= split_max / 2) hipLaunchKernelGGL((hdq_coarse_kernel<true, 8>), dim3(groups), dim3(512), 0, s, fr, rs, n, th, inv2r2, out, d, upd);
+                else hipLaunchKernelGGL((hdq_coarse_kernel<true, 4>), dim3(groups), dim3(256), 0, s, fr, rs, n, th, inv2r2, out, d, upd);
+            }
+        }
+        else if (fold) hipLaunchKernelGGL((hdq_coarse_kernel<true, 1, true, true>), grid, dim3(KNN_THREADS), 0, s, fr, rs, n, th, inv2r2, out, d, upd);
+        else if (fr.bvh_leaves > 0 && hint) hipLaunchKernelGGL((hdq_coarse_kernel<true, 1, true>), grid, dim3(KNN_THREADS), 0, s, fr, rs, n, th, inv2r2, out, d, upd);
+        else if (fr.bvh_leaves > 0) hipLaunchKernelGGL((hdq_coarse_kernel<true, 1>), grid, dim3(KNN_THREADS), 0, s, fr, rs, n, th, inv2r2, out, d, upd);
+        else hipLaunchKernelGGL((hdq_coarse_kernel<false, 1>), grid, dim3(KNN_THREADS), 0, s, fr, rs, n, th, inv2r2, out, d, upd);
         if (pass == 0) hipMemsetAsync(out.fine_count, 0, sizeof(int), s);
     }
 }
diff --git a/relightableavatar_amd/csrc/ra_kernels.hpp b/relightableavatar_amd/csrc/ra_kernels.hpp
--- a/relightableavatar_amd/csrc/ra_kernels.hpp
+++ b/relightableavatar_amd/csrc/ra_kernels.hpp
@@ -48,8 +48,6 @@
 void launch_bvh_build(const float4* pverts4, int n_verts, int* order, float* leaves, float4* sbox, int n_leaves, int n_supers, hipStream_t s);
 int bvh_leaf_count(int n_verts);
 int bvh_super_count(int n_leaves);
-void launch_hdq_coarse(const FrameState& fr, const RaySet& rs, int n, float th, float blend_radius, const HdqOut& out,
-                       hipStream_t s, bool geodesic = true);
 
 struct TraceState {
     float *t, *d0, *dt, *st, *ot, *cd, *occ, *off, *rlx;
@@ -58,6 +56,15 @@
     const int* light;
     unsigned char* stuck;
 };
+struct RayUpdate {
+    TraceState ts;
+    const float* sdf;
+    int iter;
+    ra_trace_params p;
+};
+bool hdq_coarse_folds(const FrameState& fr, const RaySet& rs, const RayUpdate& update);
+void launch_hdq_coarse(const FrameState& fr, const RaySet& rs, int n, float th, float blend_radius, const HdqOut& out,
+                       hipStream_t s, bool geodesic = true, const RayUpdate* update = nullptr);
 void launch_trace_init(const TraceState& ts, int n, const int* n_dev, const ra_trace_params& p, hipStream_t s);
 
 void launch_trace_update(const TraceState& ts, const float* sdf, int n, const int* n_dev, int iter,
@@ -104,6 +111,8 @@
     int* ray_slot;
     float *near_, *far_;
     int* ray_count;
+    TraceState init;
+    float init_offset, init_relax;
 };
 void launch_key_lights(const float* probes, int n, int ph, int pw, const float* ldir, const float* area, int L, float share, int kmax,
                        int accumulate, float* smax, unsigned char* key, hipStream_t s);
@@ -117,6 +126,8 @@
 size_t sort_hits_temp_bytes(int P);
 int launch_sort_hits(const float* surf, const float* acc, int P, const float* bbox_min, unsigned* keys_in, unsigned* keys_out,
                      int* vals_in, int* hit_idx_out, void* temp, size_t temp_bytes, hipStream_t s);
+void launch_shadow_finish(const TraceState& ts, const float* sdf, const int* ray_slot, const int* ray_count, int max_rays, int iter,
+                          const ra_trace_params& p, float* lvis, unsigned long long* n_rays, hipStream_t s);
 void launch_shadow_scatter(const float* occ, const int* ray_slot, const int* ray_count, int max_rays, float* lvis, hipStream_t s);
 
 struct ShadeIn {
diff --git a/relightableavatar_amd/csrc/ra_trace.hip b/relightableavatar_amd/csrc/ra_trace.hip
--- a/relightableavatar_amd/csrc/ra_trace.hip
+++ b/relightableavatar_amd/csrc/ra_trace.hip
@@ -1,5 +1,6 @@
 #include "ra_kernels.hpp"
 #include "ra_shade_dev.hpp"
+#include "ra_trace_step.hpp"
 #include <hipcub/hipcub.hpp>
 
 namespace {
@@ -35,62 +36,18 @@
                                     ra_trace_params p) {
     const int i = blockIdx.x * TPB + threadIdx.x;
     if (i >= live_count(n_dev, n_launch)) return;
-    const float d1 = sdf[i];
-    const float d0 = ts.d0[i];
-    float t = ts.t[i];
-    const float t_prev = t;
-    float occ = ts.occ[i];
-    const float nr = ts.near_[i], fr = ts.far_[i];
-    float tan_i = p.tan_i;
-    if (SOFT) {
-        const float ti = ts.tan_i ? (ts.light ? ts.tan_i[ts.light[i]] : ts.tan_i[i]) : p.tan_i;
-        tan_i = p.tan_i_multiplier * ti;
-    }
-    const float tan2 = (1.f / tan_i) * 2.f;
-    float off = ts.off ? ts.off[i] : p.offset;
-    float rlx = ts.rlx ? ts.rlx[i] : p.relax;
-    float ot = ts.ot ? ts.ot[i] : 0.f;
-    if (SOFT && p.clay_book && iter >= p.shadow_skip_iter) {
-        const float dx0 = d0 + rlx * d0 + off;
-        const float dx1 = d1 + rlx * d1 + off;
-        const float dy = (dx1 * dx1) / (2.f * dx0);
-        const float dx = (sqrtf(dx1 * dx1 - dy * dy) - off) / (1.f + rlx);
-        const float den = fmaxf(fmaxf(t - dy, nr), p.eps);
-        const float cls = fmaxf(dx, 0.f) / den / tan2;
-        const bool msk = (cls < occ) && (dy < t) && (dx1 > 0.f) && (dx0 > 0.f) && (dx > 0.f) && (dy > 0.f) && (dy < dx0);
-        if (msk) { ot = t - dy; occ = cls; }
-    }
-    if (iter >= p.shadow_skip_iter) {
-        const float cls = fmaxf(d1, 0.f) / fmaxf(fmaxf(t, nr), p.eps) / tan2;
-        if (cls < occ) { ot = t; occ = cls; }
-    }
-    if (!SOFT) {
-        const float d1u = fabsf(d1), d0u = fabsf(d0);
-        float st = ts.st[i], cd = ts.cd[i];
-        const float dt = ts.dt[i];
-        const float s0 = (d0 > 0.f) ? 1.f : ((d0 < 0.f) ? -1.f : 0.f);
-        const float s1 = (d1 > 0.f) ? 1.f : ((d1 < 0.f) ? -1.f : 0.f);
-        if (s0 != s1) {
-            st = t - dt * fminf(fmaxf(d1u / (d0u + d1u + p.eps), 0.f), 1.f);
-            off = 0.f;
-            rlx = 0.f;
-        }
-        if (d1u < cd) { cd = d1u; st = t; }
-        ts.st[i] = st;
-        ts.cd[i] = cd;
-        ts.off[i] = off;
-        ts.rlx[i] = rlx;
-    }
-    const float dtn = d1 + rlx * d1 + off;
-    t = t + dtn;
-    t = fminf(t, fr);
-    t = fmaxf(t, nr);
-    if (ts.dt) ts.dt[i] = dtn;
-    ts.t[i] = t;
-    if (ts.stuck) ts.stuck[i] = (t == t_prev || (SOFT && occ == 0.f)) ? 1 : 0;
-    ts.d0[i] = d1;
-    ts.occ[i] = occ;
-    if (ts.ot) ts.ot[i] = ot;
+    const TraceStepOut r = trace_step<SOFT>(ts, sdf, i, iter, p);
+    trace_step_store<SOFT>(ts, i, r);
+}
+
+template <bool SOFT>
+__global__ void shadow_finish_kernel(TraceState ts, const float* __restrict__ sdf, const int* __restrict__ ray_slot,
+                                     const int* __restrict__ ray_count, int max_rays, int iter, ra_trace_params p, float* __restrict__ lvis,
+                                     unsigned long long* __restrict__ n_rays) {
+    const int i = blockIdx.x * TPB + threadIdx.x;
+    if (i == 0) atomicAdd(n_rays, (unsigned long long)*ray_count);
+    if (i >= min(*ray_count, max_rays)) return;
+    lvis[ray_slot[i]] = trace_step<SOFT>(ts, sdf, i, iter, p).occ;
 }
 
 __global__ void surface_finish_kernel(const float* __restrict__ ro, const float* __restrict__ rd, const float* __restrict__ st,
@@ -408,6 +365,19 @@
             g.ray_slot[s] = h * g.L + l;
             g.near_[s] = nrv[round];
             g.far_[s] = frv[round];
+            if (g.init.t) {
+                const TraceState& ts = g.init;
+                ts.t[s] = nrv[round];
+                ts.d0[s] = 1e9f;
+                ts.occ[s] = 1.f;
+                if (ts.stuck) ts.stuck[s] = 0;
+                if (ts.dt) ts.dt[s] = 1e9f;
+                if (ts.st) ts.st[s] = frv[round];
+                if (ts.ot) ts.ot[s] = frv[round];
+                if (ts.cd) ts.cd[s] = 1e9f;
+                if (ts.off) ts.off[s] = g.init_offset;
+                if (ts.rlx) ts.rlx[s] = g.init_relax;
+            }
         }
     }
     const int col = threadIdx.x & (SG_LIGHTS - 1), l = lc * SG_LIGHTS + col;
@@ -1238,6 +1208,13 @@
     hipLaunchKernelGGL(shadow_scatter_kernel, grid_for(max_rays), dim3(TPB), 0, s, occ, ray_slot, ray_count, max_rays, lvis);
 }
 
+void launch_shadow_finish(const TraceState& ts, const float* sdf, const int* ray_slot, const int* ray_count, int max_rays, int iter,
+                          const ra_trace_params& p, float* lvis, unsigned long long* n_rays, hipStream_t s) {
+    if (max_rays <= 0) { launch_accumulate(ray_count, n_rays, s); return; }
+    if (p.soft_shadow) hipLaunchKernelGGL(shadow_finish_kernel<true>, grid_for(max_rays), dim3(TPB), 0, s, ts, sdf, ray_slot, ray_count, max_rays, iter, p, lvis, n_rays);
+    else hipLaunchKernelGGL(shadow_finish_kernel<false>, grid_for(max_rays), dim3(TPB), 0, s, ts, sdf, ray_slot, ray_count, max_rays, iter, p, lvis, n_rays);
+}
+
 void launch_shade(const ShadeIn& in, const ra_config& cfg, hipStream_t s) {
     if (in.n <= 0) return;
     hipLaunchKernelGGL(shade_kernel, grid_for((long long)in.n * 64), dim3(TPB), 0, s, in, cfg);
diff --git a/relightableavatar_amd/csrc/ra_trace_step.hpp b/relightableavatar_amd/csrc/ra_trace_step.hpp
--- /dev/null
+++ b/relightableavatar_amd/csrc/ra_trace_step.hpp
@@ -0,0 +1,81 @@
+#pragma once
+#include "ra_kernels.hpp"
+
+struct TraceStepOut {
+    float t, d0, dt, occ, ot, st, cd, off, rlx;
+    unsigned char stuck;
+};
+
+template <bool SOFT>
+__device__ __forceinline__ TraceStepOut trace_step(const TraceState& ts, const float* __restrict__ sdf, int i, int iter, const ra_trace_params& p) {
+#pragma clang fp contract(off)
+    TraceStepOut r;
+    const float d1 = sdf[i];
+    const float d0 = ts.d0[i];
+    float t = ts.t[i];
+    const float t_prev = t;
+    float occ = ts.occ[i];
+    const float nr = ts.near_[i], fr = ts.far_[i];
+    float tan_i = p.tan_i;
+    if (SOFT) {
+        const float ti = ts.tan_i ? (ts.light ? ts.tan_i[ts.light[i]] : ts.tan_i[i]) : p.tan_i;
+        tan_i = p.tan_i_multiplier * ti;
+    }
+    const float tan2 = (1.f / tan_i) * 2.f;
+    float off = ts.off ? ts.off[i] : p.offset;
+    float rlx = ts.rlx ? ts.rlx[i] : p.relax;
+    float ot = ts.ot ? ts.ot[i] : 0.f;
+    if (SOFT && p.clay_book && iter >= p.shadow_skip_iter) {
+        const float dx0 = fmaf(rlx, d0, d0) + off;
+        const float dx1 = fmaf(rlx, d1, d1) + off;
+        const float q1 = dx1 * dx1;
+        const float dy = q1 / (2.f * dx0);
+        const float dx = (sqrtf(fmaf(-dy, dy, q1)) - off) / (1.f + rlx);
+        const float den = fmaxf(fmaxf(t - dy, nr), p.eps);
+        const float cls = fmaxf(dx, 0.f) / den / tan2;
+        const bool msk = (cls < occ) && (dy < t) && (dx1 > 0.f) && (dx0 > 0.f) && (dx > 0.f) && (dy > 0.f) && (dy < dx0);
+        if (msk) { ot = t - dy; occ = cls; }
+    }
+    if (iter >= p.shadow_skip_iter) {
+        const float cls = fmaxf(d1, 0.f) / fmaxf(fmaxf(t, nr), p.eps) / tan2;
+        if (cls < occ) { ot = t; occ = cls; }
+    }
+    r.st = 0.f; r.cd = 0.f;
+    if (!SOFT) {
+        const float d1u = fabsf(d1), d0u = fabsf(d0);
+        float st = ts.st[i], cd = ts.cd[i];
+        const float dt = ts.dt[i];
+        const float s0 = (d0 > 0.f) ? 1.f : ((d0 < 0.f) ? -1.f : 0.f);
+        const float s1 = (d1 > 0.f) ? 1.f : ((d1 < 0.f) ? -1.f : 0.f);
+        if (s0 != s1) {
+            st = fmaf(-dt, fminf(fmaxf(d1u / (d0u + d1u + p.eps), 0.f), 1.f), t);
+            off = 0.f;
+            rlx = 0.f;
+        }
+        if (d1u < cd) { cd = d1u; st = t; }
+        r.st = st; r.cd = cd;
+    }
+    const float dtn = fmaf(rlx, d1, d1) + off;
+    t = t + dtn;
+    t = fminf(t, fr);
+    t = fmaxf(t, nr);
+    r.stuck = (t == t_prev || (SOFT && occ == 0.f)) ? 1 : 0;
+    r.t = t; r.d0 = d1; r.dt = dtn; r.occ = occ; r.ot = ot; r.off = off; r.rlx = rlx;
+    return r;
+}
+
+template <bool SOFT>
+__device__ __forceinline__ void trace_step_store(const TraceState& ts, int i, const TraceStepOut& r) {
+    if (!SOFT) {
+        ts.st[i] = r.st;
+        ts.cd[i] = r.cd;
+        ts.off[i] = r.off;
+        ts.rlx[i] = r.rlx;
+    }
+    if (ts.dt) ts.dt[i] = r.dt;
+    ts.t[i] = r.t;
+    if (ts.stuck) ts.stuck[i] = r.stuck;
+    ts.d0[i] = r.d0;
+    ts.occ[i] = r.occ;
+    if (ts.ot) ts.ot[i] = r.ot;
+}
diff --git a/relightableavatar_amd/engine.py b/relightableavatar_amd/engine.py
--- a/relightableavatar_amd/engine.py
+++ b/relightableavatar_amd/engine.py
@@ -504,6 +504,9 @@
         check(self.lib.ra_set_knn_mode(self.ctx, int(use_bvh)), 'ra_set_knn_mode')
         self._frame_key = None
 
+    def set_lvis_schedule(self, mode=2):
+        check(self.lib.ra_set_lvis_schedule(self.ctx, int(mode)), 'ra_set_lvis_schedule')
+
     def gen_rays(self, H, W, K, R, T, bounds, count=None):
         bufs, cnt = self._gen_rays(H, W, K, R, T, bounds, host_count=count is None)
         P = cnt if count is None else int(count)
```
